# s-esposito/MonoGS

Measured on AMD Instinct MI355X. Metric: rasteriser fwd+bwd Mpix/s @1080p, higher is better.
Workload: dtype f32; 1 GPU; C5: 2000000 Gaussians, 1920x1080, fwd+bwd, seeded synthetic map (SURVEY.md 8d), one keyframe per GPU; gaussians=2000000, width=1920, height=1080, settle_steps=60, instance_count=device-side (capacity mode, overflow checked), parallelism=keyframe-per-gpu x1

## Files before the change

### include/monogs_raster.h

```cpp
#ifndef MONOGS_RASTER_H
#define MONOGS_RASTER_H

#include <stddef.h>
#include <stdint.h>

#ifdef __cplusplus
extern "C" {
#endif

#define MGS_ABI_VERSION 10
#define MGS_TILE 16

typedef struct mgs_camera {
    int32_t image_height;
    int32_t image_width;
    float tanfovx;
    float tanfovy;
    float scale_modifier;
    int32_t sh_degree;
    int32_t sh_coeffs;
    int32_t scale_dim;
    int32_t flags;
    const float* bg;
    const float* viewmatrix;
    const float* projmatrix;
    const float* projmatrix_raw;
    const float* campos;
} mgs_camera;

#define MGS_FLAG_EXCLUSIVE_DEVICE 1

typedef struct mgs_timing {
    float preprocess_ms;
    float depth_sort_ms;
    float scan_ms;
    float duplicate_ms;
    float sort_ms;
    float ranges_ms;
    float blend_fwd_ms;
    float blend_bwd_ms;
    float geom_bwd_ms;
} mgs_timing;

int mgs_abi_version(void);
const char* mgs_last_error(void);

#define MGS_MAX_GAUSSIANS ((1 << 26) - 1)

size_t mgs_geometry_bytes(int32_t P);
size_t mgs_image_bytes(int32_t width, int32_t height);
size_t mgs_binning_bytes(uint64_t num_rendered, int32_t width, int32_t height);
size_t mgs_backward_bytes(int32_t P);
float* mgs_backward_tau(void* backward_scratch, int32_t P);

int mgs_forward_preprocess(const mgs_camera* cam, int32_t P,
                           const float* means3D,
                           const float* shs,
                           const float* colors_precomp,
                           const float* opacities,
                           const float* scales,
                           const float* rotations,
                           const float* cov3D_precomp,
                           void* geometry, int32_t* radii ,
                           void* prepare_backward ,
                           uint64_t* num_rendered ,
                           const uint32_t* prev_status ,
                           uint32_t* prev_status_out ,
                           mgs_timing* timing , void* stream);

int mgs_forward_render(const mgs_camera* cam, int32_t P, uint64_t num_rendered,
                       void* geometry, void* binning, void* image,
                       float* out_color, float* out_depth, float* out_opacity, int32_t* n_touched,
                       uint32_t* status ,
                       mgs_timing* timing, void* stream);

#define MGS_STATUS_CAPACITY_OVERFLOW 1u
#define MGS_STATUS_DEPTH_SORT_TIMEOUT 2u
#define MGS_STATUS_TILE_SORT_TIMEOUT 4u

int mgs_debug_set_radix_spin_limit(uint32_t limit);
int mgs_debug_set_option(const char* name, int64_t value);

int mgs_binning_path(int32_t P, int32_t W, int32_t H);

size_t mgs_debug_sort_temp_bytes(uint64_t n, int32_t bits);
int mgs_debug_sort_pairs(uint32_t* keys, uint32_t* vals, uint32_t* keys_alt, uint32_t* vals_alt, uint64_t n, int32_t bits,
                         void* temp, void* stream);

int mgs_forward_render_capacity(const mgs_camera* cam, int32_t P, uint64_t capacity,
                                void* geometry, void* binning, void* image,
                                float* out_color, float* out_depth, float* out_opacity, int32_t* n_touched,
                                uint32_t* overflow, mgs_timing* timing, void* stream);
int mgs_forward_capacity(const mgs_camera* cam, int32_t P, const float* means3D, const float* shs,
                         const float* colors_precomp, const float* opacities, const float* scales, const float* rotations,
                         const float* cov3D_precomp, void* geometry, int32_t* radii, void* prepare_backward,
                         uint64_t capacity, void* binning, void* image, float* out_color, float* out_depth,
                         float* out_opacity, int32_t* n_touched, uint32_t* overflow, mgs_timing* timing, void* stream);

int mgs_backward(const mgs_camera* cam, int32_t P, uint64_t num_rendered,
                 const float* means3D, const float* shs, const float* colors_precomp,
                 const float* opacities, const float* scales, const float* rotations,
                 const float* cov3D_precomp, const int32_t* radii,
                 const void* geometry, const void* binning, const void* image,
                 const float* dL_dcolor, const float* dL_ddepth,
                 float* dL_dmeans2D,
                 float* dL_dcolors,
                 float* dL_dopacity,
                 float* dL_dmeans3D,
                 float* dL_dcov3D,
                 float* dL_dsh,
                 float* dL_dscales,
                 float* dL_drotations,
                 float* dL_dtau,
                 void* backward_scratch, int32_t scratch_prepared, mgs_timing* timing, void* stream);

#define MGS_VALU_CEILING_BLOCKS 2048
int mgs_debug_valu_ceiling(float* out, int32_t iters, void* stream);

int mgs_debug_set_blend_events(void* fwd_start, void* fwd_end, void* bwd_start, void* bwd_end);

#define MGS_BLEND_STATS_WORDS 24
int mgs_debug_blend_stats(const mgs_camera* cam, int32_t P, uint64_t num_rendered, const void* geometry,
                          const void* binning, const void* image, uint64_t* stats_dev, void* stream);

int mgs_mark_visible(int32_t P, const float* means3D, const float* viewmatrix, const float* projmatrix,
                     uint8_t* visible, void* stream);

size_t mgs_knn_scratch_bytes(int32_t P);
int mgs_dist2_knn(int32_t P, const float* points , float* out ,
                  void* scratch, void* stream);

#define MGS_LOSS_TRACKING 1
#define MGS_LOSS_INVERT_DEPTH 2
#define MGS_LOSS_SCRATCH_DAB 10
#define MGS_LOSS_SCRATCH_LOSS 12
size_t mgs_loss_scratch_bytes(void);
int mgs_loss_forward(int32_t width, int32_t height, int32_t mode, int32_t init, float lambda_rgb,
                     const float* render, const float* depth, const float* opacity, const float* gt_rgb,
                     const float* gt_depth, const uint8_t* mask, const uint8_t* grad_mask,
                     const float* exposure_a, const float* exposure_b, float* scratch, float* loss_out,
                     void* stream);
int mgs_loss_backward(int32_t width, int32_t height, int32_t mode, int32_t init, float lambda_rgb,
                      const float* render, const float* depth, const float* opacity, const float* gt_rgb,
                      const float* gt_depth, const uint8_t* mask, const uint8_t* grad_mask,
                      const float* exposure_a, const float* exposure_b, const float* scratch,
                      const float* grad_out, float* d_render, float* d_depth, float* d_exposure, void* stream);
int mgs_loss_grads(int32_t width, int32_t height, int32_t mode, int32_t init, float lambda_rgb,
                   const float* render, const float* depth, const float* opacity, const float* gt_rgb,
                   const float* gt_depth, const uint8_t* mask, const uint8_t* grad_mask,
                   const float* exposure_a, const float* exposure_b, float* scratch, float* d_render, float* d_depth,
                   void* stream);

#define MGS_POSE_STICKY 1
int mgs_pose_step(float* R, float* T, float* rot_delta, float* trans_delta, float* exposure_a, float* exposure_b,
                  const float* grad_rot, const float* grad_trans, const float* grad_a, const float* grad_b,
                  float* adam_m, float* adam_v, int32_t step, float lr_rot, float lr_trans, float lr_exposure,
                  float beta1, float beta2, float eps, float converged_threshold, int32_t* step_counter, float* out,
                  int32_t flags, float* host_flag ,
                  const float* projmatrix_raw, float* viewmatrix, float* projmatrix, float* campos ,
                  void* stream);
int mgs_pose_step_batch(int32_t n, void* const* ptrs, float lr_rot, float lr_trans, float lr_exposure, float beta1,
                        float beta2, float eps, float converged_threshold, int32_t flags, void* stream);

int mgs_backproject(int32_t N, int32_t W, int32_t H, const int64_t* selected, const float* rgb ,
                    const float* depth , const int32_t* segmentation ,
                    const float* exposure_a, const float* exposure_b, float fx, float fy, float cx, float cy,
                    const float* R, const float* T, float* points , float* features ,
                    int32_t* ids , void* stream);

int mgs_camera_setup(const float* R, const float* T, const float* projmatrix_raw, float* viewmatrix ,
                     float* projmatrix , float* campos , void* stream);

int mgs_adam_step(int32_t n_tensors, float* const* params, const float* const* grads, float* const* exp_avg,
                  float* const* exp_avg_sq, const uint64_t* numel, const float* lr, double beta1, double beta2,
                  double eps, int32_t step, int32_t* step_counter,
                  const float* lr_device ,
                  void* stream);
int mgs_densify_stats(int32_t P, const float* viewspace_grad , const int32_t* radii,
                      float* xyz_gradient_accum , float* denom , float* max_radii_2d ,
                      void* stream);
int mgs_window_stats(int32_t P, int32_t n_keyframes, const float* const* grad_means2D, const int32_t* const* radii,
                     const int32_t* const* n_touched, float* grad_norm , float* visible ,
                     float* max_radii , int32_t accumulate, uint64_t* visibility_bits, void* stream);
int mgs_window_apply(int32_t P, const float* grad_norm, const float* visible, const float* max_radii,
                     float* xyz_gradient_accum, float* denom, float* max_radii_2d, void* stream);
int mgs_lr_schedule_step(int32_t* iteration, float* lr_out, double lr_init, double lr_final, int32_t lr_delay_steps,
                         double lr_delay_mult, int32_t max_steps, void* stream);

int mgs_activate_forward(int32_t P, int32_t scale_dim , const float* rot_raw ,
                         const float* scale_raw , const float* opacity_raw ,
                         float* rotations , float* scales3 , float* opacities ,
                         void* stream);
int mgs_activate_backward(int32_t P, int32_t scale_dim, const float* rot_raw, const float* scales3,
                          const float* opacities, const float* grad_rotations, const float* grad_scales3,
                          const float* grad_opacities, float* d_rot_raw, float* d_scale_raw, float* d_opacity_raw,
                          void* stream);

int mgs_sum_buffers(int32_t n_src, const float* const* src, float* dst, uint64_t count, void* stream);

#ifdef __cplusplus
}
#endif
#endif
```

### monogs_amd/_lib.py

```python
from __future__ import annotations

import ctypes as C
import os

_HERE = os.path.dirname(os.path.abspath(__file__))
LIB_PATH = os.environ.get("MGS_LIB_PATH") or os.path.join(_HERE, "lib", "libmonogs_raster.so")
ABI_VERSION = 10

c_float_p = C.c_void_p


class MgsCamera(C.Structure):
    _fields_ = [
        ("image_height", C.c_int32), ("image_width", C.c_int32),
        ("tanfovx", C.c_float), ("tanfovy", C.c_float), ("scale_modifier", C.c_float),
        ("sh_degree", C.c_int32), ("sh_coeffs", C.c_int32), ("scale_dim", C.c_int32), ("flags", C.c_int32),
        ("bg", C.c_void_p), ("viewmatrix", C.c_void_p), ("projmatrix", C.c_void_p),
        ("projmatrix_raw", C.c_void_p), ("campos", C.c_void_p),
    ]


class MgsTiming(C.Structure):
    _fields_ = [(n, C.c_float) for n in (
        "preprocess_ms", "depth_sort_ms", "scan_ms", "duplicate_ms", "sort_ms", "ranges_ms", "blend_fwd_ms",
        "blend_bwd_ms", "geom_bwd_ms")]

    def as_dict(self):
        return {n: float(getattr(self, n)) for n, _ in self._fields_}


SIGNATURES = {
    "mgs_abi_version": (C.c_int, []),
    "mgs_last_error": (C.c_char_p, []),
    "mgs_geometry_bytes": (C.c_size_t, [C.c_int32]),
    "mgs_image_bytes": (C.c_size_t, [C.c_int32, C.c_int32]),
    "mgs_binning_bytes": (C.c_size_t, [C.c_uint64, C.c_int32, C.c_int32]),
    "mgs_backward_bytes": (C.c_size_t, [C.c_int32]),
    "mgs_forward_preprocess": (C.c_int, [C.POINTER(MgsCamera), C.c_int32] + [C.c_void_p] * 7
                               + [C.c_void_p, C.c_void_p, C.c_void_p, C.POINTER(C.c_uint64), C.c_void_p, C.POINTER(C.c_uint32),
                                  C.POINTER(MgsTiming), C.c_void_p]),
    "mgs_forward_capacity": (C.c_int, [C.POINTER(MgsCamera), C.c_int32] + [C.c_void_p] * 7 + [C.c_void_p] * 3 + [C.c_uint64]
                             + [C.c_void_p] * 7 + [C.POINTER(MgsTiming), C.c_void_p]),
    "mgs_forward_render": (C.c_int, [C.POINTER(MgsCamera), C.c_int32, C.c_uint64] + [C.c_void_p] * 8
                           + [C.POINTER(MgsTiming), C.c_void_p]),
    "mgs_debug_set_radix_spin_limit": (C.c_int, [C.c_uint32]),
    "mgs_debug_set_option": (C.c_int, [C.c_char_p, C.c_int64]),
    "mgs_binning_path": (C.c_int, [C.c_int32, C.c_int32, C.c_int32]),
    "mgs_debug_sort_temp_bytes": (C.c_size_t, [C.c_uint64, C.c_int32]),
    "mgs_debug_sort_pairs": (C.c_int, [C.c_void_p] * 4 + [C.c_uint64, C.c_int32, C.c_void_p, C.c_void_p]),
    "mgs_forward_render_capacity": (C.c_int, [C.POINTER(MgsCamera), C.c_int32, C.c_uint64] + [C.c_void_p] * 8
                                    + [C.POINTER(MgsTiming), C.c_void_p]),
    "mgs_backward": (C.c_int, [C.POINTER(MgsCamera), C.c_int32, C.c_uint64] + [C.c_void_p] * 7
                     + [C.c_void_p] * 4 + [C.c_void_p] * 2 + [C.c_void_p] * 9
                     + [C.c_void_p, C.c_int32, C.POINTER(MgsTiming), C.c_void_p]),
    "mgs_backward_tau": (C.c_void_p, [C.c_void_p, C.c_int32]),
    "mgs_debug_blend_stats": (C.c_int, [C.POINTER(MgsCamera), C.c_int32, C.c_uint64] + [C.c_void_p] * 5),
    "mgs_debug_valu_ceiling": (C.c_int, [C.c_void_p, C.c_int32, C.c_void_p]),
    "mgs_debug_set_blend_events": (C.c_int, [C.c_void_p] * 4),
    "mgs_mark_visible": (C.c_int, [C.c_int32, C.c_void_p, C.c_void_p, C.c_void_p, C.c_void_p, C.c_void_p]),
    "mgs_loss_scratch_bytes": (C.c_size_t, []),
    "mgs_loss_forward": (C.c_int, [C.c_int32] * 4 + [C.c_float] + [C.c_void_p] * 9 + [C.c_void_p, C.c_void_p, C.c_void_p]),
    "mgs_loss_backward": (C.c_int, [C.c_int32] * 4 + [C.c_float] + [C.c_void_p] * 9
                          + [C.c_void_p, C.c_void_p, C.c_void_p, C.c_void_p, C.c_void_p, C.c_void_p]),
    "mgs_loss_grads": (C.c_int, [C.c_int32] * 4 + [C.c_float] + [C.c_void_p] * 9 + [C.c_void_p] * 4),
    "mgs_backproject": (C.c_int, [C.c_int32] * 3 + [C.c_void_p] * 6 + [C.c_float] * 4 + [C.c_void_p] * 6),
    "mgs_camera_setup": (C.c_int, [C.c_void_p] * 7),
    "mgs_pose_step": (C.c_int, [C.c_void_p] * 12 + [C.c_int32] + [C.c_float] * 7
                      + [C.c_void_p, C.c_void_p, C.c_int32, C.c_void_p] + [C.c_void_p] * 4 + [C.c_void_p]),
    "mgs_pose_step_batch": (C.c_int, [C.c_int32, C.POINTER(C.c_void_p)] + [C.c_float] * 7 + [C.c_int32, C.c_void_p]),
    "mgs_adam_step": (C.c_int, [C.c_int32] + [C.c_void_p] * 6 + [C.c_double] * 3 + [C.c_int32, C.c_void_p, C.c_void_p, C.c_void_p]),
    "mgs_window_stats": (C.c_int, [C.c_int32, C.c_int32] + [C.c_void_p] * 6 + [C.c_int32, C.c_void_p, C.c_void_p]),
    "mgs_window_apply": (C.c_int, [C.c_int32] + [C.c_void_p] * 7),
    "mgs_lr_schedule_step": (C.c_int, [C.c_void_p, C.c_void_p, C.c_double, C.c_double, C.c_int32, C.c_double, C.c_int32, C.c_void_p]),
    "mgs_densify_stats": (C.c_int, [C.c_int32] + [C.c_void_p] * 6),
    "mgs_sum_buffers": (C.c_int, [C.c_int32, C.POINTER(C.c_void_p), C.c_void_p, C.c_uint64, C.c_void_p]),
    "mgs_activate_forward": (C.c_int, [C.c_int32, C.c_int32] + [C.c_void_p] * 7),
    "mgs_activate_backward": (C.c_int, [C.c_int32, C.c_int32] + [C.c_void_p] * 10),
    "mgs_knn_scratch_bytes": (C.c_size_t, [C.c_int32]),
    "mgs_dist2_knn": (C.c_int, [C.c_int32, C.c_void_p, C.c_void_p, C.c_void_p, C.c_void_p]),
}

_lib = None


class MonoGSNativeError(RuntimeError):
    pass


def load():
    global _lib
    if _lib is not None:
        return _lib
    if not os.path.exists(LIB_PATH):
        raise MonoGSNativeError(
            f"{LIB_PATH} not found: build it with `python -c 'import __graft_entry__ as g; g.build()'` "
            "or `make -C monogs_amd/csrc`.  There is no CPU fallback.")
    lib = C.CDLL(LIB_PATH)
    for name, (res, args) in SIGNATURES.items():
        fn = getattr(lib, name)
        fn.restype = res
        fn.argtypes = args
    if lib.mgs_abi_version() != ABI_VERSION:
        raise MonoGSNativeError(f"ABI mismatch: library {lib.mgs_abi_version()} vs binding {ABI_VERSION}; rebuild")
    for kv in filter(None, os.environ.get("MGS_DEBUG_OPTIONS", "").split(",")):
        k, _, v = kv.partition("=")
        if lib.mgs_debug_set_option(k.strip().encode(), int(v)) != 0:
            raise MonoGSNativeError(f"MGS_DEBUG_OPTIONS: {lib.mgs_last_error().decode()}")
    _lib = lib
    return lib


def check(rc: int, what: str):
    if rc != 0:
        msg = load().mgs_last_error().decode("utf-8", "replace")
        raise Exception(msg) if rc == 1 else MonoGSNativeError(f"{what}: {msg}")
```

### monogs_amd/csrc/api.hip

```cpp
#include "common.h"

#include <stdarg.h>
#include <stdio.h>
#include <string.h>

namespace mgs {

static thread_local char g_err[512] = "";

void set_error(const char* fmt, ...) {
    va_list ap;
    va_start(ap, fmt);
    vsnprintf(g_err, sizeof(g_err), fmt, ap);
    va_end(ap);
}

static inline char* take(char*& p, size_t bytes) {
    char* r = p;
    p += align_up(bytes, 256);
    return r;
}

GeometryState GeometryState::carve(void* base, int P) {
    char* p = (char*)align_up((size_t)base, 256);
    GeometryState g;
    g.rec = (float*)take(p, (size_t)P * REC_FLOATS * sizeof(float));
    g.depth_key = (uint32_t*)take(p, (size_t)P * sizeof(uint32_t));
    g.depth_alt = (uint32_t*)take(p, (size_t)P * sizeof(uint32_t));
    g.iota = (uint32_t*)take(p, (size_t)P * sizeof(uint32_t));
    g.iota_alt = (uint32_t*)take(p, (size_t)P * sizeof(uint32_t));
    g.perm = (uint32_t*)take(p, (size_t)P * sizeof(uint32_t));
    g.point_offsets = (uint32_t*)take(p, (size_t)P * sizeof(uint32_t));
    g.scan_blocks = (uint32_t*)take(p, ((size_t)scan_nblocks(P) + 64) * sizeof(uint32_t));
    g.clamped = (uint8_t*)take(p, (size_t)P * 4);
    g.rect = (uint2*)take(p, (size_t)P * sizeof(uint2));
    g.rect_sorted = (uint2*)take(p, (size_t)P * sizeof(uint2));
    g.scan_status = (uint64_t*)take(p, (SCAN_SMALL_MAX_BLOCKS + 1) * sizeof(uint64_t));
    g.tile_hist = (uint32_t*)take(p, 4 * 256 * sizeof(uint32_t));
    g.sort_temp_bytes = radix_depth_temp_bytes((uint64_t)P);
    g.sort_temp = take(p, g.sort_temp_bytes);
    g.end = p;
    return g;
}
size_t GeometryState::bytes(int P) {
    const GeometryState g = carve(nullptr, P);
    return (size_t)g.end + 256;
}

size_t ImageState::bytes(int W, int H) {
    const size_t HW = (size_t)W * H, nt = (size_t)tiles_x(W) * tiles_y(H);
    return align_up(HW * 4, 256) * 2 + align_up(nt * sizeof(uint2), 256) + 256;
}
ImageState ImageState::carve(void* base, int W, int H) {
    const size_t HW = (size_t)W * H, nt = (size_t)tiles_x(W) * tiles_y(H);
    char* p = (char*)align_up((size_t)base, 256);
    ImageState s;
    s.final_T = (float*)take(p, HW * 4);
    s.n_contrib = (uint32_t*)take(p, HW * 4);
    s.ranges = (uint2*)take(p, nt * sizeof(uint2));
    return s;
}

size_t BinningState::bytes(uint64_t R, int W, int H) {
    const size_t r = (size_t)(R ? R : 1);
    return align_up(r * 4, 256) * 4 + align_up(mgs::sort_temp_bytes(R, tile_bits(W, H)), 256) + 256 + 256;
}
BinningState BinningState::carve(void* base, uint64_t R, int W, int H) {
    const size_t r = (size_t)(R ? R : 1);
    char* p = (char*)align_up((size_t)base, 256);
    BinningState b;
    b.keys_a = (uint32_t*)take(p, r * 4);
    b.keys_b = (uint32_t*)take(p, r * 4);
    b.vals_a = (uint32_t*)take(p, r * 4);
    b.vals_b = (uint32_t*)take(p, r * 4);
    const bool in_b = radix_result_in_b(tile_bits(W, H));
    b.keys_sorted = in_b ? b.keys_b : b.keys_a;
    b.vals_sorted = in_b ? b.vals_b : b.vals_a;
    b.sort_temp_bytes = mgs::sort_temp_bytes(R, tile_bits(W, H));
    b.sort_temp = take(p, b.sort_temp_bytes);
    b.count = (uint32_t*)take(p, 2 * sizeof(uint32_t));
    return b;
}

struct StageTimer {
    hipStream_t s;
    bool on;
    hipEvent_t ev[10];
    int n = 0;
    StageTimer(hipStream_t s_, bool on_) : s(s_), on(on_) {
        if (on) for (auto& e : ev) (void)hipEventCreate(&e);
    }
    ~StageTimer() {
        if (on) for (auto& e : ev) (void)hipEventDestroy(e);
    }
    void mark() {
        if (on && n < 10) (void)hipEventRecord(ev[n++], s);
    }
    float ms(int i) {
        float t = 0.f;
        if (on && i + 1 < n) (void)hipEventElapsedTime(&t, ev[i], ev[i + 1]);
        return t;
    }
    void sync() {
        if (on && n) (void)hipEventSynchronize(ev[n - 1]);
    }
};

static int check_cam(const mgs_camera* cam) {
    if (!cam) { set_error("camera is NULL"); return 1; }
    if (cam->image_width <= 0 || cam->image_height <= 0) { set_error("image size must be positive"); return 1; }
    if (!cam->bg || !cam->viewmatrix || !cam->projmatrix || !cam->projmatrix_raw || !cam->campos) {
        set_error("camera tensors (bg, viewmatrix, projmatrix, projmatrix_raw, campos) must be non-NULL");
        return 1;
    }
    return 0;
}

static hipEvent_t g_dbg_fwd_events[2] = {nullptr, nullptr}, g_dbg_bwd_events[2] = {nullptr, nullptr};

static int check_map_size(int32_t P) {
    if (P > MGS_MAX_GAUSSIANS) {
        set_error("P exceeds MGS_MAX_GAUSSIANS (2^26 - 1): the gradient-line offset of the blend backward is 32-bit");
        return 1;
    }
    return 0;
}

}

using namespace mgs;

extern "C" {

int mgs_abi_version(void) { return MGS_ABI_VERSION; }
int mgs_binning_path(int32_t P, int32_t W, int32_t H) { return binning_path(P, W, H); }
const char* mgs_last_error(void) { return g_err; }

size_t mgs_geometry_bytes(int32_t P) { return GeometryState::bytes(P < 0 ? 0 : P); }
size_t mgs_image_bytes(int32_t W, int32_t H) { return ImageState::bytes(W, H); }
size_t mgs_binning_bytes(uint64_t R, int32_t W, int32_t H) { return BinningState::bytes(R, W, H); }
size_t mgs_backward_bytes(int32_t P) {
    return (size_t)(P < 0 ? 0 : P) * GRAD_FLOATS * sizeof(float) + (size_t)(TAU_SLOTS + 1) * 16 * sizeof(float) + 256;
}
float* mgs_backward_tau(void* backward_scratch, int32_t P) { return backward_tau_out(backward_scratch, P < 0 ? 0 : P); }

int mgs_forward_preprocess(const mgs_camera* cam, int32_t P, const float* means3D, const float* shs,
                           const float* colors_precomp, const float* opacities, const float* scales,
                           const float* rotations, const float* cov3D_precomp, void* geometry, int32_t* radii,
                           void* prepare_backward, uint64_t* num_rendered, const uint32_t* prev_status,
                           uint32_t* prev_status_out, mgs_timing* timing, void* stream) {
    if (check_cam(cam)) return 1;
    if (P < 0) { set_error("P must be >= 0"); return 1; }
    if (check_map_size(P)) return 1;
    if (num_rendered) *num_rendered = 0;
    if (prev_status_out) *prev_status_out = 0;
    if (P == 0) {
        if (prev_status && prev_status_out) {
            MGS_HIP(hipMemcpyAsync(prev_status_out, prev_status, sizeof(uint32_t), hipMemcpyDeviceToHost, (hipStream_t)stream));
            MGS_HIP(hipStreamSynchronize((hipStream_t)stream));
        }
        return 0;
    }
    if (!means3D || !opacities || !geometry || !radii) { set_error("means3D, opacities, geometry, radii must be non-NULL"); return 1; }
    if ((shs == nullptr) == (colors_precomp == nullptr)) {
        set_error("Please provide excatly one of either SHs or precomputed colors!");
        return 1;
    }
    const bool have_sr = scales != nullptr || rotations != nullptr;
    if ((have_sr && (!scales || !rotations || cov3D_precomp)) || (!have_sr && !cov3D_precomp)) {
        set_error("Please provide exactly one of either scale/rotation pair or precomputed 3D covariance!");
        return 1;
    }
    if (shs && (cam->sh_degree < 0 || cam->sh_degree > 3 || cam->sh_coeffs < (cam->sh_degree + 1) * (cam->sh_degree + 1))) {
        set_error("sh_degree must be 0..3 and shs must hold at least (degree+1)^2 coefficients");
        return 1;
    }
    hipStream_t s = (hipStream_t)stream;
    GeometryState g = GeometryState::carve(geometry, P);
    StageTimer tm(s, timing != nullptr);
    tm.mark();
    if (int rc = launch_preprocess_forward(*cam, P, means3D, shs, colors_precomp, opacities, scales, rotations,
                                           cov3D_precomp, g, radii,
                                           prepare_backward ? backward_grad_acc(prepare_backward) : nullptr, s)) return rc;
    tm.mark();
    const bool exclusive = (cam->flags & MGS_FLAG_EXCLUSIVE_DEVICE) != 0;
    const bool per_tile = binning_path(P, cam->image_width, cam->image_height) != 0;
    if (per_tile) {
        tm.mark();
        if (int rc = launch_scan(g, P, s, exclusive, g.rect)) return rc;
    } else if (depth_chain_is_small(P)) {
        if (int rc = launch_depth_chain_small(g, P, s)) return rc;
        tm.mark();
    } else {
        if (int rc = launch_depth_sort(g, P, depth_sort_payload(P, cam->image_width, cam->image_height), s, exclusive)) return rc;
        tm.mark();
        if (int rc = launch_scan(g, P, s, exclusive, g.rect_sorted)) return rc;
    }
    tm.mark();
    if (num_rendered) {
        uint32_t total = 0, sort_errors[RADIX_ERROR_WORDS] = {0, 0, 0, 0};
        MGS_HIP(hipMemcpyAsync(&total, g.scan_blocks + scan_nblocks(P), sizeof(uint32_t), hipMemcpyDeviceToHost, s));
        MGS_HIP(hipMemcpyAsync(sort_errors, radix_depth_error_flag(g.sort_temp, (uint64_t)P), sizeof(sort_errors),
                               hipMemcpyDeviceToHost, s));
        if (prev_status && prev_status_out)
            MGS_HIP(hipMemcpyAsync(prev_status_out, prev_status, sizeof(uint32_t), hipMemcpyDeviceToHost, s));
        MGS_HIP(hipStreamSynchronize(s));
        if (sort_errors[0] | sort_errors[1] | sort_errors[2] | sort_errors[3]) { set_error("depth sort: a look-back spin timed out (results invalid)"); return 3; }
        *num_rendered = total;
    }
    if (timing) {
        if (!num_rendered) MGS_HIP(hipStreamSynchronize(s));
        timing->preprocess_ms = tm.ms(0);
        timing->depth_sort_ms = per_tile ? 0.f : tm.ms(1);
        timing->scan_ms = tm.ms(2);
    }
    return 0;
}

static int g_opt_tile_sort_fused = 1;

static int forward_render_impl(const mgs_camera* cam, int32_t P, uint64_t R, bool capacity, void* geometry,
                               void* binning, void* image, float* out_color, float* out_depth, float* out_opacity,
                               int32_t* n_touched, uint32_t* overflow, mgs_timing* timing, void* stream) {
    if (check_cam(cam)) return 1;
    if (P < 0) { set_error("P must be >= 0"); return 1; }
    if (check_map_size(P)) return 1;
    if (!image || !out_color || !out_depth || !out_opacity) { set_error("image scratch and outputs must be non-NULL"); return 1; }
    if (P > 0 && (!geometry || !n_touched)) { set_error("geometry and n_touched must be non-NULL"); return 1; }
    if (R > 0 && !binning) { set_error("binning scratch is NULL"); return 1; }
    if (R >= (1ull << 32)) { set_error("num_rendered exceeds 2^32-1"); return 1; }
    if (P == 0) R = 0;
    hipStream_t s = (hipStream_t)stream;
    const int W = cam->image_width, H = cam->image_height;
    GeometryState g = GeometryState::carve(geometry, P);
    ImageState img = ImageState::carve(image, W, H);
    BinningState b = BinningState::carve(binning, R, W, H);
    const uint32_t* n_dev = nullptr;
    StageTimer tm(s, timing != nullptr);
    const bool cap = capacity && binning;
    if (cap) n_dev = b.count;
    const bool per_tile = binning_path(P, W, H) != 0;
    tm.mark();
    if (int rc = launch_duplicate(*cam, P, g, b, capacity ? R : (R > 0 ? 0xFFFFFFFFull : 0ull), n_touched, img, R,
                                  tile_bits(W, H), cap ? b.count : nullptr, overflow, s, per_tile)) return rc;
    tm.mark();
    if (int rc = launch_sort(g, b, R, tile_bits(W, H), s, n_dev, (cam->flags & MGS_FLAG_EXCLUSIVE_DEVICE) != 0, img.ranges,
                             per_tile)) return rc;
    const uint32_t* sort_err = R > 0 ? radix_error_flag(b.sort_temp, R, tile_bits(W, H)) : nullptr;
    const bool sort_tiles = per_tile && R > 0;
    const TileSortArgs ts = sort_tiles ? tile_sort_args(*cam, g, b, R, n_dev) : TileSortArgs{};
    const bool fused = sort_tiles && g_opt_tile_sort_fused != 0;
    if (sort_tiles && !fused)
        if (int rc = launch_tile_depth_sort(*cam, ts, img, sort_err, s)) return rc;
    tm.mark();
    if (g_dbg_fwd_events[0]) MGS_HIP(hipEventRecord(g_dbg_fwd_events[0], s));
    if (int rc = launch_blend_forward(*cam, g, b, img, out_color, out_depth, out_opacity, n_touched, sort_err, overflow,
                                      fused ? &ts : nullptr, s)) return rc;
    if (g_dbg_fwd_events[1]) MGS_HIP(hipEventRecord(g_dbg_fwd_events[1], s));
    tm.mark();
    if (timing) {
        tm.sync();
        timing->duplicate_ms = tm.ms(0);
        timing->sort_ms = tm.ms(1);
        timing->ranges_ms = 0.f;
        timing->blend_fwd_ms = tm.ms(2);
    }
    return 0;
}

int mgs_forward_render(const mgs_camera* cam, int32_t P, uint64_t R, void* geometry, void* binning, void* image,
                       float* out_color, float* out_depth, float* out_opacity, int32_t* n_touched,
                       uint32_t* status, mgs_timing* timing, void* stream) {
    return forward_render_impl(cam, P, R, false, geometry, binning, image, out_color, out_depth, out_opacity, n_touched,
                               status, timing, stream);
}

int mgs_forward_render_capacity(const mgs_camera* cam, int32_t P, uint64_t capacity, void* geometry, void* binning,
                                void* image, float* out_color, float* out_depth, float* out_opacity,
                                int32_t* n_touched, uint32_t* overflow, mgs_timing* timing, void* stream) {
    if (capacity == 0) { set_error("capacity must be > 0"); return 1; }
    return forward_render_impl(cam, P, capacity, true, geometry, binning, image, out_color, out_depth, out_opacity,
                               n_touched, overflow, timing, stream);
}

int mgs_forward_capacity(const mgs_camera* cam, int32_t P, const float* means3D, const float* shs,
                         const float* colors_precomp, const float* opacities, const float* scales, const float* rotations,
                         const float* cov3D_precomp, void* geometry, int32_t* radii, void* prepare_backward,
                         uint64_t capacity, void* binning, void* image, float* out_color, float* out_depth,
                         float* out_opacity, int32_t* n_touched, uint32_t* overflow, mgs_timing* timing, void* stream) {
    if (int rc = mgs_forward_preprocess(cam, P, means3D, shs, colors_precomp, opacities, scales, rotations, cov3D_precomp,
                                        geometry, radii, prepare_backward, nullptr, nullptr, nullptr, timing, stream)) return rc;
    return mgs_forward_render_capacity(cam, P, capacity, geometry, binning, image, out_color, out_depth, out_opacity,
                                       n_touched, overflow, timing, stream);
}

int mgs_backward(const mgs_camera* cam, int32_t P, uint64_t R, const float* means3D, const float* shs,
                 const float* colors_precomp, const float* opacities, const float* scales, const float* rotations,
                 const float* cov3D_precomp, const int32_t* radii, const void* geometry, const void* binning,
                 const void* image, const float* dL_dcolor, const float* dL_ddepth, float* dL_dmeans2D,
                 float* dL_dcolors, float* dL_dopacity, float* dL_dmeans3D, float* dL_dcov3D, float* dL_dsh,
                 float* dL_dscales, float* dL_drotations, float* dL_dtau, void* backward_scratch,
                 int32_t scratch_prepared, mgs_timing* timing, void* stream) {
    if (check_cam(cam)) return 1;
    if (P < 0) { set_error("P must be >= 0"); return 1; }
    if (check_map_size(P)) return 1;
    hipStream_t s = (hipStream_t)stream;
    if (P == 0) {
        if (dL_dtau) MGS_HIP(zero_fill(dL_dtau, 6 * sizeof(float), s));
        return 0;
    }
    if (!means3D || !opacities || !radii || !geometry || !image || !dL_dcolor || !dL_ddepth || !backward_scratch) {
        set_error("means3D, opacities, radii, geometry, image, dL_dcolor, dL_ddepth, backward_scratch must be non-NULL");
        return 1;
    }
    if (R > 0 && !binning) { set_error("binning scratch is NULL"); return 1; }
    const int W = cam->image_width, H = cam->image_height;
    GeometryState g = GeometryState::carve(const_cast<void*>(geometry), P);
    ImageState img = ImageState::carve(const_cast<void*>(image), W, H);
    BinningState b = BinningState::carve(const_cast<void*>(binning), R, W, H);
    float* grad_acc = backward_grad_acc(backward_scratch);
    StageTimer tm(s, timing != nullptr);
    float* tau_part = (dL_dtau && (P + 255) / 256 > TAU_DIRECT_MAX_BLOCKS) ? backward_tau_part(backward_scratch, P) : nullptr;
    if (scratch_prepared) {
        if (dL_dtau && dL_dtau != backward_tau_out(backward_scratch, P)) {
            set_error("scratch_prepared: dL_dtau must be mgs_backward_tau(backward_scratch, P)");
            return 1;
        }
    } else {
        MGS_HIP(zero_fill2(grad_acc, (size_t)P * GRAD_FLOATS * sizeof(float) + (tau_part ? (size_t)TAU_SLOTS * 16 * sizeof(float) : 0),
                           dL_dtau, 6 * sizeof(float), s));
    }
    tm.mark();
    if (R > 0) {
        const bool pose_only = !dL_dcolors && !dL_dopacity && !dL_dsh && !shs;
        if (g_dbg_bwd_events[0]) MGS_HIP(hipEventRecord(g_dbg_bwd_events[0], s));
        if (int rc = launch_blend_backward(*cam, g, b, img, dL_dcolor, dL_ddepth, grad_acc, pose_only, s)) return rc;
        if (g_dbg_bwd_events[1]) MGS_HIP(hipEventRecord(g_dbg_bwd_events[1], s));
    }
    tm.mark();
    GeomBackwardArgs a;
    a.means3D = means3D; a.shs = shs; a.colors_precomp = colors_precomp; a.opacities = opacities;
    a.scales = scales; a.rotations = rotations; a.cov3D_precomp = cov3D_precomp; a.radii = radii;
    a.grad_acc = grad_acc;
    a.dL_dmeans2D = dL_dmeans2D; a.dL_dcolors = dL_dcolors; a.dL_dopacity = dL_dopacity;
    a.dL_dmeans3D = dL_dmeans3D; a.dL_dcov3D = dL_dcov3D; a.dL_dsh = dL_dsh; a.dL_dscales = dL_dscales;
    a.dL_drotations = dL_drotations; a.dL_dtau = dL_dtau; a.tau_part = tau_part;
    if (int rc = launch_geom_backward(*cam, P, g, a, s)) return rc;
    tm.mark();
    if (timing) {
        tm.sync();
        timing->blend_bwd_ms = tm.ms(0);
        timing->geom_bwd_ms = tm.ms(1);
    }
    return 0;
}

int mgs_debug_blend_stats(const mgs_camera* cam, int32_t P, uint64_t R, const void* geometry, const void* binning,
                           const void* image, uint64_t* stats_dev, void* stream) {
    if (check_cam(cam)) return 1;
    if (!geometry || !image || !stats_dev || (R > 0 && !binning)) { set_error("bad arguments"); return 1; }
    hipStream_t s = (hipStream_t)stream;
    MGS_HIP(zero_fill(stats_dev, MGS_BLEND_STATS_WORDS * sizeof(uint64_t), s));
    if (P == 0 || R == 0) return 0;
    const int W = cam->image_width, H = cam->image_height;
    GeometryState g = GeometryState::carve(const_cast<void*>(geometry), P);
    ImageState img = ImageState::carve(const_cast<void*>(image), W, H);
    BinningState b = BinningState::carve(const_cast<void*>(binning), R, W, H);
    return launch_blend_backward_stats(*cam, g, b, img, (unsigned long long*)stats_dev, s);
}

int mgs_debug_valu_ceiling(float* out, int32_t iters, void* stream) {
    if (!out || iters < 1) { set_error("mgs_debug_valu_ceiling: bad arguments"); return 1; }
    return launch_valu_ceiling(out, iters, (hipStream_t)stream);
}

int mgs_debug_set_radix_spin_limit(uint32_t limit) { return set_radix_spin_limit(limit); }

int mgs_debug_set_blend_events(void* fwd_start, void* fwd_end, void* bwd_start, void* bwd_end) {
    if ((fwd_start == nullptr) != (fwd_end == nullptr) || (bwd_start == nullptr) != (bwd_end == nullptr)) {
        set_error("mgs_debug_set_blend_events: a pair is both events or neither");
        return 1;
    }
    g_dbg_fwd_events[0] = (hipEvent_t)fwd_start; g_dbg_fwd_events[1] = (hipEvent_t)fwd_end;
    g_dbg_bwd_events[0] = (hipEvent_t)bwd_start; g_dbg_bwd_events[1] = (hipEvent_t)bwd_end;
    return 0;
}

static int g_opt_debug_sort_exclusive = 0;
size_t mgs_debug_sort_temp_bytes(uint64_t n, int32_t bits) { return radix_temp_bytes(n, bits); }
int mgs_debug_sort_pairs(uint32_t* keys, uint32_t* vals, uint32_t* keys_alt, uint32_t* vals_alt, uint64_t n, int32_t bits,
                         void* temp, void* stream) {
    if (bits < 1 || bits > 32 || (n && (!keys || !vals || !keys_alt || !vals_alt || !temp))) {
        set_error("mgs_debug_sort_pairs: bad arguments");
        return 1;
    }
    if (n == 0) return 0;
    hipStream_t s = (hipStream_t)stream;
    if (int rc = radix_sort_pairs(keys, vals, keys_alt, vals_alt, n, bits, temp, s, nullptr, false, nullptr, nullptr, nullptr, false,
                                  g_opt_debug_sort_exclusive != 0))
        return rc;
    if (radix_result_in_b(bits)) {
        MGS_HIP(hipMemcpyAsync(keys, keys_alt, n * 4, hipMemcpyDeviceToDevice, s));
        MGS_HIP(hipMemcpyAsync(vals, vals_alt, n * 4, hipMemcpyDeviceToDevice, s));
    }
    uint32_t err[RADIX_ERROR_WORDS];
    MGS_HIP(hipMemcpyAsync(err, radix_error_flag(temp, n, bits), sizeof(err), hipMemcpyDeviceToHost, s));
    MGS_HIP(hipStreamSynchronize(s));
    if (err[0] | err[1] | err[2] | err[3]) { set_error("mgs_debug_sort_pairs: a look-back spin timed out"); return 2; }
    return 0;
}

int mgs_debug_set_option(const char* name, int64_t value) {
    if (name && !strcmp(name, "radix_scanned")) { g_opt_radix_scanned = (int)value; return 0; }
    if (name && !strcmp(name, "radix_ballot_rank")) { g_opt_radix_ballot_rank = (int)value; return 0; }
    if (name && !strcmp(name, "radix_tile_items")) { g_opt_radix_tile_items = (int)value; return 0; }
    if (name && !strcmp(name, "radix_xcd_band")) { g_opt_radix_xcd_band = (int)value; return 0; }
    if (name && !strcmp(name, "debug_sort_exclusive")) { g_opt_debug_sort_exclusive = (int)value; return 0; }
    if (name && !strcmp(name, "dup_slot_major")) { g_opt_dup_slot_major = (int)value; return 0; }
    if (name && !strcmp(name, "blend_bwd_transposed")) { g_opt_blend_bwd_transposed = (int)value; return 0; }
    if (name && !strcmp(name, "scan_small")) { g_opt_scan_small = (int)value; return 0; }
    if (name && !strcmp(name, "depth_small")) { g_opt_depth_small = (int)value; return 0; }
    if (name && !strcmp(name, "tile_sort_fused")) { g_opt_tile_sort_fused = value < 0 ? 1 : (int)value; return 0; }
    if (name && !strcmp(name, "blend_lds_pad_fwd")) { g_opt_blend_lds_pad_fwd = (int)value; return 0; }
    if (name && !strcmp(name, "blend_lds_pad_bwd")) { g_opt_blend_lds_pad_bwd = (int)value; return 0; }
    if (name && !strcmp(name, "knn_grid_min")) { g_opt_knn_grid_min = value > 0x7FFFFFFF ? 0x7FFFFFFF : (int)value; return 0; }
    set_error("mgs_debug_set_option: unknown option");
    return 1;
}

int mgs_mark_visible(int32_t P, const float* means3D, const float* viewmatrix, const float* projmatrix,
                     uint8_t* visible, void* stream) {
    (void)projmatrix;
    if (P < 0 || (P > 0 && (!means3D || !viewmatrix || !visible))) { set_error("bad arguments"); return 1; }
    return launch_mark_visible(P, means3D, viewmatrix, visible, (hipStream_t)stream);
}

size_t mgs_knn_scratch_bytes(int32_t P) { return knn_scratch_bytes(P); }

int mgs_dist2_knn(int32_t P, const float* points, float* out, void* scratch, void* stream) {
    if (P < 0 || (P > 0 && (!points || !out))) { set_error("bad arguments"); return 1; }
    return launch_knn(P, points, out, scratch, (hipStream_t)stream);
}

}
```

### monogs_amd/csrc/blend.hip

```cpp
#include "common.h"
#include "tile_sort.h"

#include <type_traits>


namespace mgs {

extern int g_opt_blend_lds_pad_fwd, g_opt_blend_lds_pad_bwd;
#ifdef BS_TRACE
static unsigned long long* g_trace_fwd = nullptr;
static unsigned long long* g_trace_bwd = nullptr;
#define BS_STAMP(v) asm volatile("s_memrealtime %0\n\ts_waitcnt lgkmcnt(0)" : "=s"(v) :: "memory")
#endif

__device__ __forceinline__ uint32_t bcast(uint32_t v, int lane) {
    return (uint32_t)__builtin_amdgcn_readlane((int)v, lane);
}

constexpr int MGS_WG_WAVES = 4;
#define MGS_TILE_WAVE(ntiles_, tile_, wave_, ws_)                                                   \
    const int tile_ = (int)blockIdx.x, wave_ = __builtin_amdgcn_readfirstlane((int)(threadIdx.x >> 6)), ws_ = wave_; \
    if (tile_ >= (ntiles_)) return;
struct BlendArgs {
#ifdef BS_TRACE
    unsigned long long* trace;
#endif
    const float4* __restrict__ rec;
    const uint32_t* __restrict__ point_list;
    const uint2* __restrict__ ranges;
    const float* __restrict__ bg;
    int W, H, gx;
};

__device__ __forceinline__ bool quadrant_hit(const float4 c , const float4 n ,
                                             float qx0, float qy0, unsigned long long alive) {
    const float x0 = qx0 - 0.05f - c.x, x1 = qx0 + (float)(SUB - 1) + 0.05f - c.x;
    const float y0 = qy0 - 0.05f - c.y, y1 = qy0 + (float)(SUB - 1) + 0.05f - c.y;
    if (c.z < 0.f) return false;
    if (!((c.z >= x0) && (-c.z <= x1) && (c.w >= y0) && (-c.w <= y1))) return false;
    {
        const int ix0 = (int)fminf(8.f, fmaxf(0.f, ceilf(-x0 - c.z - 0.06f))), ix1 = (int)fminf(7.f, fmaxf(-1.f, floorf(-x0 + c.z + 0.06f)));
        const int iy0 = (int)fminf(8.f, fmaxf(0.f, ceilf(-y0 - c.w - 0.06f))), iy1 = (int)fminf(7.f, fmaxf(-1.f, floorf(-y0 + c.w + 0.06f)));
        if (ix0 > ix1 || iy0 > iy1) return false;
        const unsigned long long cols = (unsigned long long)((0xFFu >> (7 - ix1)) & (0xFFu << ix0) & 0xFFu) * 0x0101010101010101ull;
        const unsigned long long rows = (~0ull >> (8 * (7 - iy1))) & (~0ull << (8 * iy0));
        if ((cols & rows & alive) == 0ull) return false;
    }
    if (x0 <= 0.f && x1 >= 0.f && y0 <= 0.f && y1 >= 0.f) return true;
    if (!(n.x > 0.f) || !(n.z > 0.f)) return true;
    const float rby = -n.y * __builtin_amdgcn_rcpf(n.z), rbx = -n.y * __builtin_amdgcn_rcpf(n.x);
    auto edge_x = [&](float xe) {
        const float t = fminf(y1, fmaxf(y0, rby * xe));
        return n.x * xe * xe + 2.f * n.y * xe * t + n.z * t * t;
    };
    auto edge_y = [&](float ye) {
        const float t = fminf(x1, fmaxf(x0, rbx * ye));
        return n.x * t * t + 2.f * n.y * t * ye + n.z * ye * ye;
    };
    const float qmin = fminf(fminf(edge_x(x0), edge_x(x1)), fminf(edge_y(y0), edge_y(y1)));
    return qmin <= 1.02f;
}

struct Rec {
    float px, py, ca, cb, cc, op, r, g, b, z;
};
__device__ __forceinline__ Rec fetch(const BlendArgs& a, uint32_t gid_uniform) {
    const const_float_p p = MGS_CONST(reinterpret_cast<const float*>(a.rec)) + (size_t)gid_uniform * REC_FLOATS;
    return Rec{p[R_X], p[R_Y], p[R_CA], p[R_CB], p[R_CC], p[R_OPAC], p[R_R], p[R_G], p[R_B], p[R_DEPTH]};
}

#ifdef MGS_FWD_SCALAR
#define MGS_RECOP "s"
#else
#define MGS_RECOP "v"
#endif
template <bool TOUCH>
__device__ __forceinline__ void blend_one(unsigned long long& live, unsigned long long& mask, float& T, uint32_t& last, float& C0, float& C1, float& C2,
                                      float& D, const Rec& g, float power, float alpha, uint32_t pos, int j,
                                      int& touched_cnt) {
    const float test_T = T * (1.f - alpha);
    float w;
    int cnt;
    if (TOUCH) {
        asm volatile(
            "s_mov_b64 exec, %[live]\n\t"
            "v_cmpx_nlt_f32_e32 vcc, 0, %[power]\n\t"
            "v_cmpx_ngt_f32_e32 vcc, %[amin], %[alpha]\n\t"
            "v_cmp_gt_f32_e32 vcc, %[tmin], %[tt]\n\t"
            "s_andn2_b64 exec, exec, vcc\n\t"
            "s_andn2_b64 %[live], %[live], vcc\n\t"
            "s_cselect_b64 %[mask], %[mask], 0\n\t"
            "v_mul_f32_e32 %[w], %[alpha], %[T]\n\t"
            "v_mov_b32_e32 %[T], %[tt]\n\t"
            "v_mov_b32_e32 %[last], %[pos]\n\t"
            "v_cmp_lt_f32_e32 vcc, 0.5, %[tt]\n\t"
            "v_fmac_f32_e32 %[C0], %[cr], %[w]\n\t"
            "v_fmac_f32_e32 %[C1], %[cg], %[w]\n\t"
            "s_bcnt1_i32_b64 %[cnt], vcc\n\t"
            "s_mov_b32 m0, %[j]\n\t"
            "v_fmac_f32_e32 %[C2], %[cb], %[w]\n\t"
            "v_fmac_f32_e32 %[D], %[cz], %[w]\n\t"
            "s_mov_b64 exec, -1\n\t"
            "v_writelane_b32 %[tc], %[cnt], m0\n\t"
            : [live] "+s"(live), [mask] "+s"(mask), [T] "+v"(T), [last] "+v"(last), [C0] "+v"(C0), [C1] "+v"(C1), [C2] "+v"(C2), [D] "+v"(D),
              [w] "=&v"(w), [cnt] "=&s"(cnt), [tc] "+v"(touched_cnt)
            : [power] "v"(power), [alpha] "v"(alpha), [tt] "v"(test_T), [amin] "s"(1.0f / 255.0f), [tmin] "s"(0.0001f),
              [pos] "s"(pos), [cr] MGS_RECOP(g.r), [cg] MGS_RECOP(g.g), [cb] MGS_RECOP(g.b), [cz] MGS_RECOP(g.z), [j] "s"(j)
            : "vcc", "scc", "m0");
    } else {
        asm volatile(
            "s_mov_b64 exec, %[live]\n\t"
            "v_cmpx_nlt_f32_e32 vcc, 0, %[power]\n\t"
            "v_cmpx_ngt_f32_e32 vcc, %[amin], %[alpha]\n\t"
            "v_cmp_gt_f32_e32 vcc, %[tmin], %[tt]\n\t"
            "s_andn2_b64 exec, exec, vcc\n\t"
            "s_andn2_b64 %[live], %[live], vcc\n\t"
            "s_cselect_b64 %[mask], %[mask], 0\n\t"
            "v_mul_f32_e32 %[w], %[alpha], %[T]\n\t"
            "v_mov_b32_e32 %[T], %[tt]\n\t"
            "v_mov_b32_e32 %[last], %[pos]\n\t"
            "v_fmac_f32_e32 %[C0], %[cr], %[w]\n\t"
            "v_fmac_f32_e32 %[C1], %[cg], %[w]\n\t"
            "v_fmac_f32_e32 %[C2], %[cb], %[w]\n\t"
            "v_fmac_f32_e32 %[D], %[cz], %[w]\n\t"
            "s_mov_b64 exec, -1\n\t"
            : [live] "+s"(live), [mask] "+s"(mask), [T] "+v"(T), [last] "+v"(last), [C0] "+v"(C0), [C1] "+v"(C1), [C2] "+v"(C2), [D] "+v"(D),
              [w] "=&v"(w)
            : [power] "v"(power), [alpha] "v"(alpha), [tt] "v"(test_T), [amin] "s"(1.0f / 255.0f), [tmin] "s"(0.0001f),
              [pos] "s"(pos), [cr] MGS_RECOP(g.r), [cg] MGS_RECOP(g.g), [cb] MGS_RECOP(g.b), [cz] MGS_RECOP(g.z)
            : "vcc", "scc");
    }
}

template <bool SORT>
__global__ void __launch_bounds__(256) blend_forward_kernel(BlendArgs a, float* __restrict__ out_color,
                                                            float* __restrict__ out_depth,
                                                            float* __restrict__ out_opacity,
                                                            float* __restrict__ final_T,
                                                            uint32_t* __restrict__ n_contrib,
                                                            int32_t* __restrict__ n_touched,
                                                            uint2* ranges_rw ,
                                                            const uint32_t* __restrict__ sort_err,
                                                            uint32_t* __restrict__ status, TileSortArgs ts) {
    MGS_TILE_WAVE(a.gx * ((a.H + TILE - 1) / TILE), tile, wave, ws)
    const int tx = tile % a.gx, ty = tile / a.gx;
    const int lane = threadIdx.x & 63;
    const bool first_of_tile = wave == 0 && lane == 0;
    const int qx0i = tx * TILE + (wave & 1) * SUB, qy0i = ty * TILE + (wave >> 1) * SUB;
    const int pxi = qx0i + (lane & 7), pyi = qy0i + (lane >> 3);
    const bool inside = pxi < a.W && pyi < a.H;
    const float pxf = (float)pxi, pyf = (float)pyi;
    const float qx0 = (float)qx0i, qy0 = (float)qy0i;
    uint2 range = ranges_rw[tile];
    const uint2 range_raw = range;
    const bool sort_bad = sort_err != nullptr && radix_failed(sort_err) != 0u;
    {
        if (sort_bad && tile == 0 && first_of_tile && status) atomicOr(status, (uint32_t)MGS_STATUS_TILE_SORT_TIMEOUT);
        if (sort_bad || range.x >= range.y) {
            range = make_uint2(0u, 0u);
            if (first_of_tile) ranges_rw[tile] = range;
        }
    }

    float T = 1.f, C0 = 0.f, C1 = 0.f, C2 = 0.f, D = 0.f;
    uint32_t last = 0;
    unsigned long long live = __builtin_amdgcn_ballot_w64(inside);
#ifdef BS_TRACE
    unsigned long long tr0;
    BS_STAMP(tr0);
#endif

    uint32_t gid_n = 0;
    float4 box_n = make_float4(0.f, 0.f, -1.f, -1.f), ell_n = make_float4(0.f, 0.f, 0.f, 0.f);
#ifdef MGS_FWD_SCALAR
    typedef float fv2 __attribute__((ext_vector_type(2)));
    typedef float fv8 __attribute__((ext_vector_type(8)));
    const const_float_p recs = MGS_CONST(reinterpret_cast<const float*>(a.rec));
    auto prefetch = [&](uint32_t i) {
        gid_n = 0;
        box_n = make_float4(0.f, 0.f, -1.f, -1.f);
        if (i < range.y) {
            gid_n = a.point_list[i];
            box_n = a.rec[(size_t)gid_n * 4];
            ell_n = a.rec[(size_t)gid_n * 4 + 3];
        }
    };
    auto walk_step = [&](auto touch_tag, uint32_t base, uint32_t gid_l, unsigned long long mask) {
        int touched_cnt = 0;
        const uint32_t goff_l = gid_l << 6;
        while (mask) {
            int j;
            asm volatile("s_ff1_i32_b64 %0, %1\n\ts_bitset0_b64 %1, %0" : "=&s"(j), "+s"(mask));
            const uint32_t goff = (uint32_t)__builtin_amdgcn_readlane((int)goff_l, j);
            fv2 r0;
            fv8 r1;
            asm volatile("s_load_dwordx2 %0, %2, %3\n\ts_load_dwordx8 %1, %2, %3 offset:0x10\n\ts_waitcnt lgkmcnt(0)"
                         : "=&s"(r0), "=&s"(r1) : "s"(recs), "s"(goff) : "memory");
            const Rec g{r0[0], r0[1], r1[0], r1[1], r1[2], r1[3], r1[4], r1[5], r1[6], r1[7]};
            const float dx = g.px - pxf, dy = g.py - pyf;
            const float power = dx * (g.ca * dx + g.cb * dy) + (g.cc * dy) * dy;
            const float alpha = fminf(0.99f, g.op * __builtin_amdgcn_exp2f(power));
            blend_one<decltype(touch_tag)::value>(live, mask, T, last, C0, C1, C2, D, g, power, alpha,
                                                  (base - range.x) + (uint32_t)j + 1u, j, touched_cnt);
        }
        if (decltype(touch_tag)::value && touched_cnt != 0) atomicAdd(n_touched + gid_l, touched_cnt);
    };
    if (range.x < range.y) prefetch(range.x + lane);
    for (uint32_t base = range.x; base < range.y && live != 0ull; base += WAVE) {
        const uint32_t gid_l = gid_n;
        const float4 c = box_n, el = ell_n;
        prefetch(base + WAVE + lane);
        const unsigned long long mask = __builtin_amdgcn_ballot_w64(quadrant_hit(c, el, qx0, qy0, live));
        if ((live & __builtin_amdgcn_ballot_w64(T > 0.5f)) != 0ull) walk_step(std::true_type{}, base, gid_l, mask);
        else walk_step(std::false_type{}, base, gid_l, mask);
    }
#else
    __shared__ __attribute__((aligned(16))) float4 s_queue[MGS_WG_WAVES][WAVE][3];
    __shared__ uint32_t s_list[TDS_CAP], s_wsum[TDS_WAVES], s_red[2 * TDS_WAVES];
    static_assert(sizeof(s_queue) == sizeof(uint32_t) * (TDS_CAP + TDS_WAVES * TDS_RADIX), "sort scratch = record queue");
    bool list_in_lds = false;
    if constexpr (SORT) {
        uint32_t* const s_k = reinterpret_cast<uint32_t*>(&s_queue[0][0][0]);
        const uint32_t n_lds = tile_depth_sort(ts, range_raw, sort_bad,
                                               TdsLds{s_k, s_list, reinterpret_cast<uint32_t (*)[TDS_RADIX]>(s_k + TDS_CAP),
                                                      s_wsum, s_red});
        list_in_lds = n_lds != 0u && n_lds == range.y - range.x;
        if (!list_in_lds) __syncthreads();
    }
    float4 c1_n = make_float4(0.f, 0.f, 0.f, 0.f), c2_n = c1_n;
    float4* const my_entry = &s_queue[ws][lane][0];
    const uint32_t q_base = (uint32_t)__builtin_amdgcn_readfirstlane((int)(uint32_t)(uintptr_t)&s_queue[ws][0][0]);
    auto prefetch = [&](uint32_t i) {
        gid_n = 0;
        box_n = make_float4(0.f, 0.f, -1.f, -1.f);
        if (i < range.y) {
            if constexpr (SORT) gid_n = list_in_lds ? s_list[i - range.x] : ts.vals[i];
            else gid_n = a.point_list[i];
            box_n = a.rec[(size_t)gid_n * 4];
            ell_n = a.rec[(size_t)gid_n * 4 + 3];
            c1_n = a.rec[(size_t)gid_n * 4 + 1];
            c2_n = a.rec[(size_t)gid_n * 4 + 2];
        }
    };
    auto walk_step = [&](auto touch_tag, uint32_t base, uint32_t gid_l, unsigned long long mask) {
        int touched_cnt = 0;
        while (mask) {
            const int j = __builtin_ctzll(mask);
            mask &= ~(1ull << j);
            typedef float qv2 __attribute__((ext_vector_type(2)));
            typedef float qv4 __attribute__((ext_vector_type(4)));
            qv2 e0;
            qv4 e1, e2;
            {
                const uint32_t ad = q_base + (uint32_t)j * 48u;
                asm volatile("ds_read_b64 %0, %3\n\tds_read_b128 %1, %3 offset:16\n\tds_read_b128 %2, %3 offset:32"
                             : "=&v"(e0), "=&v"(e1), "=&v"(e2) : "v"(ad) : "memory");
            }
            asm volatile("s_waitcnt lgkmcnt(2)" : "+v"(e0));
            float dx = e0[0] - pxf, dy = e0[1] - pyf;
            asm volatile("s_waitcnt lgkmcnt(1)" : "+v"(e1), "+v"(dx), "+v"(dy));
            const float power = dx * (e1[0] * dx + e1[1] * dy) + (e1[2] * dy) * dy;
            float alpha = fminf(0.99f, e1[3] * __builtin_amdgcn_exp2f(power));
            asm volatile("s_waitcnt lgkmcnt(0)" : "+v"(e2), "+v"(alpha));
            const Rec g{e0[0], e0[1], e1[0], e1[1], e1[2], e1[3], e2[0], e2[1], e2[2], e2[3]};
            blend_one<decltype(touch_tag)::value>(live, mask, T, last, C0, C1, C2, D, g, power, alpha,
                                                  (base - range.x) + (uint32_t)j + 1u, j, touched_cnt);
        }
        if (decltype(touch_tag)::value && touched_cnt != 0) atomicAdd(n_touched + gid_l, touched_cnt);
    };
    if (range.x < range.y) prefetch(range.x + lane);
    for (uint32_t base = range.x; base < range.y && live != 0ull; base += WAVE) {
        const uint32_t gid_l = gid_n;
        const float4 c = box_n, el = ell_n;
        my_entry[0] = c; my_entry[1] = c1_n; my_entry[2] = c2_n;
        prefetch(base + WAVE + lane);
        const unsigned long long mask = __builtin_amdgcn_ballot_w64(quadrant_hit(c, el, qx0, qy0, live));
        if ((live & __builtin_amdgcn_ballot_w64(T > 0.5f)) != 0ull) walk_step(std::true_type{}, base, gid_l, mask);
        else walk_step(std::false_type{}, base, gid_l, mask);
    }
#endif
#ifdef BS_TRACE
    if (a.trace) {
        unsigned long long tr1;
        BS_STAMP(tr1);
        const unsigned hw = __builtin_amdgcn_s_getreg((31 << 11) | 4), xcc = __builtin_amdgcn_s_getreg((31 << 11) | 20);
        if (lane == 0) {
            unsigned long long* o = a.trace + ((size_t)tile * 4 + wave) * 4;
            o[0] = tr0; o[1] = tr1; o[2] = (unsigned long long)hw | ((unsigned long long)xcc << 32); o[3] = range.y - range.x;
        }
    }
#endif
    if (inside) {
        const size_t pix = (size_t)pyi * a.W + pxi, HW = (size_t)a.H * a.W;
        final_T[pix] = T;
        n_contrib[pix] = last;
        out_color[pix] = C0 + T * a.bg[0];
        out_color[HW + pix] = C1 + T * a.bg[1];
        out_color[2 * HW + pix] = C2 + T * a.bg[2];
        out_depth[pix] = D;
        out_opacity[pix] = 1.f - T;
    }
}

static BlendArgs make_args(const mgs_camera& cam, const GeometryState& g, const BinningState& b,
                           const ImageState& img) {
    BlendArgs a;
#ifdef BS_TRACE
    a.trace = nullptr;
#endif
    a.rec = reinterpret_cast<const float4*>(g.rec);
    a.point_list = b.vals_sorted;
    a.ranges = img.ranges;
    a.bg = cam.bg;
    a.W = cam.image_width;
    a.H = cam.image_height;
    a.gx = tiles_x(a.W);
    return a;
}

int launch_blend_forward(const mgs_camera& cam, const GeometryState& g, const BinningState& b,
                         const ImageState& img, float* out_color, float* out_depth, float* out_opacity,
                         int32_t* n_touched, const uint32_t* sort_err, uint32_t* status, const TileSortArgs* tile_sort,
                         hipStream_t s) {
    BlendArgs a = make_args(cam, g, b, img);
#ifdef BS_TRACE
    a.trace = g_trace_fwd;
#endif
    const int ntiles = a.gx * tiles_y(a.H);
    if (ntiles == 0) return 0;
    const dim3 grid(ntiles), block(256);
    const TileSortArgs ts = tile_sort ? *tile_sort : TileSortArgs{};
#ifdef MGS_FWD_SCALAR
    if (tile_sort)
        if (int rc = launch_tile_depth_sort(cam, ts, img, sort_err, s)) return rc;
    hipLaunchKernelGGL(blend_forward_kernel<false>, grid, block, (size_t)g_opt_blend_lds_pad_fwd, s, a, out_color, out_depth,
                       out_opacity, img.final_T, img.n_contrib, n_touched, img.ranges, sort_err, status, ts);
#else
    if (tile_sort)
        hipLaunchKernelGGL(blend_forward_kernel<true>, grid, block, (size_t)g_opt_blend_lds_pad_fwd, s, a, out_color, out_depth,
                           out_opacity, img.final_T, img.n_contrib, n_touched, img.ranges, sort_err, status, ts);
    else
        hipLaunchKernelGGL(blend_forward_kernel<false>, grid, block, (size_t)g_opt_blend_lds_pad_fwd, s, a, out_color, out_depth,
                           out_opacity, img.final_T, img.n_contrib, n_touched, img.ranges, sort_err, status, ts);
#endif
    MGS_HIP(hipGetLastError());
    return 0;
}


__device__ __forceinline__ float swap32_add(float x, float y) {
    auto r = __builtin_amdgcn_permlane32_swap(__float_as_uint(x), __float_as_uint(y), false, false);
    return __uint_as_float(r[0]) + __uint_as_float(r[1]);
}
__device__ __forceinline__ float swap16_add(float x, float y) {
    auto r = __builtin_amdgcn_permlane16_swap(__float_as_uint(x), __float_as_uint(y), false, false);
    return __uint_as_float(r[0]) + __uint_as_float(r[1]);
}
template <int XOR>
__device__ __forceinline__ float swz_add(float v) {
    return v + __int_as_float(__builtin_amdgcn_ds_swizzle(__float_as_int(v), 0x001F | (XOR << 10)));
}
__device__ __forceinline__ float row_sum_all(float v) {
    v = swz_add<1>(v);
    v = swz_add<2>(v);
    v = swz_add<4>(v);
    v = swz_add<8>(v);
    return v;
}
__device__ __forceinline__ int reduce10_slot(int lane) {
    const int row = lane >> 4, pos = lane & 15;
    if (pos == 15) return row == 0 ? 0 : row == 1 ? 2 : row == 2 ? 1 : 3;
    if (pos == 0) return row == 0 ? 4 : row == 1 ? 6 : row == 2 ? 5 : 7;
    if (pos == 1) return row == 0 ? 8 : row == 2 ? 9 : -1;
    return -1;
}
__device__ __forceinline__ float reduce10(float a0, float a1, float a2, float a3, float a4, float a5, float a6,
                                          float a7, float a8, float a9, int lane) {
    const float b0 = swap32_add(a0, a1), b1 = swap32_add(a2, a3), b2 = swap32_add(a4, a5);
    const float b3 = swap32_add(a6, a7), b4 = swap32_add(a8, a9);
    float c0 = swap16_add(b0, b1);
    float c1 = swap16_add(b2, b3);
    float c2 = swz_add<16>(b4);
    c0 = row_sum_all(c0);
    c1 = row_sum_all(c1);
    c2 = row_sum_all(c2);
    const int pos = lane & 15;
    return pos == 15 ? c0 : (pos == 0 ? c1 : c2);
}

__device__ __forceinline__ int reduce6_slot(int lane) {
    const int row = lane >> 4, pos = lane & 15;
    if (pos == 15) return row == 0 ? G_SX : row == 1 ? G_SXX : row == 2 ? G_SY : G_SXY;
    if (pos == 0) return row == 0 ? G_SYY : row == 2 ? G_DDEPTH : -1;
    return -1;
}
__device__ __forceinline__ float reduce6(float a0, float a1, float a2, float a3, float a4, float a5, int lane) {
    const float b0 = swap32_add(a0, a1), b1 = swap32_add(a2, a3), b2 = swap32_add(a4, a5);
    float c0 = swap16_add(b0, b1);
    float c1 = swz_add<16>(b2);
    c0 = row_sum_all(c0);
    c1 = row_sum_all(c1);
    return (lane & 15) == 15 ? c0 : c1;
}

__device__ __forceinline__ uint32_t wave_max_u32(uint32_t v) {
#pragma unroll
    for (int o = 32; o > 0; o >>= 1) v = max(v, (uint32_t)__shfl_xor((int)v, o, 64));
    return v;
}

template <bool POSE_ONLY>
__global__ void __launch_bounds__(256) blend_backward_kernel(BlendArgs a, int ntiles,
                                                             const float* __restrict__ final_T,
                                                             const uint32_t* __restrict__ n_contrib,
                                                             const float* __restrict__ dL_dcolor,
                                                             const float* __restrict__ dL_ddepth,
                                                             float* __restrict__ grad_acc) {
    const int wave = threadIdx.x >> 6, lane = threadIdx.x & 63;
    const int tile = (int)blockIdx.x;
    if (tile >= ntiles) return;
    const int tx = tile % a.gx, ty = tile / a.gx;
    const uint2 range = a.ranges[tile];
    if (range.y <= range.x) return;
    const size_t HW = (size_t)a.H * a.W;
    const float bg0 = a.bg[0], bg1 = a.bg[1], bg2 = a.bg[2];

    const int qx0i = tx * TILE + (wave & 1) * SUB, qy0i = ty * TILE + (wave >> 1) * SUB;
    const int pxi = qx0i + (lane & 7), pyi = qy0i + (lane >> 3);
    const bool inside = pxi < a.W && pyi < a.H;
    const size_t pix = (size_t)pyi * a.W + pxi;
    const float pxf = (float)pxi, pyf = (float)pyi, qx0 = (float)qx0i, qy0 = (float)qy0i;
    const float T_final = inside ? final_T[pix] : 0.f;
    const uint32_t last = inside ? n_contrib[pix] : 0u;
    const float g0 = inside ? dL_dcolor[pix] : 0.f;
    const float g1 = inside ? dL_dcolor[HW + pix] : 0.f;
    const float g2 = inside ? dL_dcolor[2 * HW + pix] : 0.f;
    const float gd = inside ? dL_ddepth[pix] : 0.f;
    const float bgT = -T_final * (bg0 * g0 + bg1 * g1 + bg2 * g2);
    float T = T_final, Bk = 0.f;
    const uint32_t maxc = wave_max_u32(last);
    if (maxc == 0) return;
    const uint32_t end = range.x + maxc;

    const int slot = POSE_ONLY ? reduce6_slot(lane) : reduce10_slot(lane);
    const uint32_t slot_bytes = slot < 0 ? 0u : (uint32_t)slot * 4u;

    uint32_t gid_n = 0;
    float4 box_n = make_float4(0.f, 0.f, -1.f, -1.f), ell_n = make_float4(0.f, 0.f, 0.f, 0.f);
    auto prefetch = [&](int b) {
        gid_n = 0;
        box_n = make_float4(0.f, 0.f, -1.f, -1.f);
        const uint32_t i = range.x + (uint32_t)b * WAVE + lane;
        if (b >= 0 && i < end) {
            gid_n = a.point_list[i];
            box_n = a.rec[(size_t)gid_n * 4];
            ell_n = a.rec[(size_t)gid_n * 4 + 3];
        }
    };
    prefetch((int)((maxc - 1) / WAVE));
    for (int b = (int)((maxc - 1) / WAVE); b >= 0; --b) {
        const uint32_t gid_l = gid_n;
        const float4 c = box_n, el = ell_n;
        prefetch(b - 1);
        const unsigned long long alive = __builtin_amdgcn_ballot_w64(last >= (uint32_t)b * WAVE + 1u);
        unsigned long long mask = __builtin_amdgcn_ballot_w64(quadrant_hit(c, el, qx0, qy0, alive));
        const int rel_last = (int)last - (int)((uint32_t)b * WAVE + 1u);
        while (mask) {
            const int j = 63 - __builtin_clzll(mask);
            mask &= ~(1ull << j);
            const uint32_t gid = bcast(gid_l, j);
            const Rec g = fetch(a, gid);
            const float dx = g.px - pxf, dy = g.py - pyf;
            const float power = dx * (g.ca * dx + g.cb * dy) + (g.cc * dy) * dy;
            const float G = __builtin_amdgcn_exp2f(power);
            const float alpha = fminf(0.99f, g.op * G);
            const bool act = (j <= rel_last) && !(power > 0.f) && !(alpha < 1.0f / 255.0f);
            if (__builtin_amdgcn_ballot_w64(act) == 0ull) continue;
            const float a_eff = act ? alpha : 0.f;
            const float inv = __builtin_amdgcn_rcpf(1.f - a_eff);
            const float Tn = T * inv;
            const float qq = __builtin_fmaf(g.z, gd, __builtin_fmaf(g.b, g2, __builtin_fmaf(g.g, g1, g.r * g0)));
            const float diff = qq - Bk;
            const float dL_dalpha = diff * Tn + bgT * inv;
            Bk = Bk + a_eff * diff;
            T = Tn;
            const float w = a_eff * Tn;
            const float h = act ? G * dL_dalpha : 0.f;
            const float hx = h * dx, hy = h * dy;
            const float s_x = hx, s_y = hy, s_xx = hx * dx, s_xy = hx * dy, s_yy = hy * dy, s_h = h;
            const float s_r = w * g0, s_g = w * g1, s_b = w * g2, s_z = w * gd;
            const float m = POSE_ONLY ? reduce6(s_x, s_y, s_xx, s_xy, s_yy, s_z, lane)
                                      : reduce10(s_x, s_y, s_xx, s_xy, s_yy, s_h, s_r, s_g, s_b, s_z, lane);
            float* const line = grad_acc + (size_t)gid * GRAD_FLOATS;
            if (slot >= 0) asm volatile("global_atomic_add_f32 %0, %1, %2" ::"v"(slot_bytes), "v"(m), "s"(line) : "memory");
        }
    }
}

constexpr int BT_SLOTS = 4;
constexpr int BS_STRIDE = 272;
constexpr int BS_W_OFF = 1280;
constexpr int BS_META_OFF = BS_W_OFF + BT_SLOTS * BS_STRIDE;
__device__ __forceinline__ int bt_slot10(int t) {
    const int bank = t >> 2, m = t & 3;
    if (m == 0) return bank == 3 ? 0 : bank == 1 ? 1 : bank == 2 ? 2 : 3;
    if (m == 1) return bank == 3 ? 4 : bank == 1 ? 5 : bank == 2 ? 6 : 7;
    if (m == 2) return bank == 3 ? 8 : bank == 1 ? 9 : -1;
    return -1;
}
__device__ __forceinline__ int bt_slot6(int t) {
    const int bank = t >> 2, m = t & 3;
    if (m == 0) return bank == 3 ? G_SX : bank == 1 ? G_SY : bank == 2 ? G_SXX : G_SXY;
    if (m == 1) return bank == 3 ? G_SYY : bank == 1 ? G_DDEPTH : -1;
    return -1;
}
__device__ __forceinline__ float reduce_rows10(float v0, float v1, float v2, float v3, float v4, float v5, float v6,
                                               float v7, float v8, float v9, unsigned long long m1, unsigned long long m2) {
    float a0, a1, a2, a3, a4;
    asm volatile(
        "s_nop 1\n\t"
        "v_add_f32_dpp %0, %5, %5 row_ror:8 row_mask:0xf bank_mask:0xc\n\t"
        "v_add_f32_dpp %1, %7, %7 row_ror:8 row_mask:0xf bank_mask:0xc\n\t"
        "v_add_f32_dpp %2, %9, %9 row_ror:8 row_mask:0xf bank_mask:0xc\n\t"
        "v_add_f32_dpp %3, %11, %11 row_ror:8 row_mask:0xf bank_mask:0xc\n\t"
        "v_add_f32_dpp %4, %13, %13 row_ror:8 row_mask:0xf bank_mask:0xc\n\t"
        "v_add_f32_dpp %0, %6, %6 row_ror:8 row_mask:0xf bank_mask:0x3\n\t"
        "v_add_f32_dpp %1, %8, %8 row_ror:8 row_mask:0xf bank_mask:0x3\n\t"
        "v_add_f32_dpp %2, %10, %10 row_ror:8 row_mask:0xf bank_mask:0x3\n\t"
        "v_add_f32_dpp %3, %12, %12 row_ror:8 row_mask:0xf bank_mask:0x3\n\t"
        "v_add_f32_dpp %4, %14, %14 row_ror:8 row_mask:0xf bank_mask:0x3\n\t"
        "v_add_f32_dpp %5, %0, %0 row_half_mirror row_mask:0xf bank_mask:0xa\n\t"
        "v_add_f32_dpp %6, %2, %2 row_half_mirror row_mask:0xf bank_mask:0xa\n\t"
        "v_add_f32_dpp %5, %1, %1 row_half_mirror row_mask:0xf bank_mask:0x5\n\t"
        "v_add_f32_dpp %6, %3, %3 row_half_mirror row_mask:0xf bank_mask:0x5\n\t"
        "v_add_f32_dpp %7, %4, %4 row_half_mirror row_mask:0xf bank_mask:0xf\n\t"
        "v_add_f32_dpp %0, %5, %5 quad_perm:[2,3,0,1] row_mask:0xf bank_mask:0xf\n\t"
        "v_add_f32_dpp %1, %6, %6 quad_perm:[2,3,0,1] row_mask:0xf bank_mask:0xf\n\t"
        "v_add_f32_dpp %2, %7, %7 quad_perm:[2,3,0,1] row_mask:0xf bank_mask:0xf\n\t"
        "v_add_f32_dpp %5, %0, %0 quad_perm:[1,0,3,2] row_mask:0xf bank_mask:0xf\n\t"
        "v_add_f32_dpp %6, %1, %1 quad_perm:[1,0,3,2] row_mask:0xf bank_mask:0xf\n\t"
        "v_add_f32_dpp %7, %2, %2 quad_perm:[1,0,3,2] row_mask:0xf bank_mask:0xf\n\t"
        : "=&v"(a0), "=&v"(a1), "=&v"(a2), "=&v"(a3), "=&v"(a4), "+v"(v0), "+v"(v1), "+v"(v2), "+v"(v3), "+v"(v4), "+v"(v5),
          "+v"(v6), "+v"(v7), "+v"(v8), "+v"(v9));
    const float r12 = __builtin_amdgcn_inverse_ballot_w64(m1) ? v1 : v2;
    return __builtin_amdgcn_inverse_ballot_w64(m2) ? v0 : r12;
}
__device__ __forceinline__ float reduce_rows6(float v0, float v1, float v2, float v3, float v4, float v5,
                                              unsigned long long m2) {
    float a0, a1, a2;
    asm volatile(
        "s_nop 1\n\t"
        "v_add_f32_dpp %0, %3, %3 row_ror:8 row_mask:0xf bank_mask:0xc\n\t"
        "v_add_f32_dpp %1, %5, %5 row_ror:8 row_mask:0xf bank_mask:0xc\n\t"
        "v_add_f32_dpp %2, %7, %7 row_ror:8 row_mask:0xf bank_mask:0xc\n\t"
        "v_add_f32_dpp %0, %4, %4 row_ror:8 row_mask:0xf bank_mask:0x3\n\t"
        "v_add_f32_dpp %1, %6, %6 row_ror:8 row_mask:0xf bank_mask:0x3\n\t"
        "v_add_f32_dpp %2, %8, %8 row_ror:8 row_mask:0xf bank_mask:0x3\n\t"
        "v_add_f32_dpp %3, %0, %0 row_half_mirror row_mask:0xf bank_mask:0xa\n\t"
        "v_add_f32_dpp %3, %1, %1 row_half_mirror row_mask:0xf bank_mask:0x5\n\t"
        "v_add_f32_dpp %4, %2, %2 row_half_mirror row_mask:0xf bank_mask:0xf\n\t"
        "s_nop 1\n\t"
        "v_add_f32_dpp %0, %3, %3 quad_perm:[2,3,0,1] row_mask:0xf bank_mask:0xf\n\t"
        "v_add_f32_dpp %1, %4, %4 quad_perm:[2,3,0,1] row_mask:0xf bank_mask:0xf\n\t"
        "s_nop 0\n\t"
        "v_add_f32_dpp %3, %0, %0 quad_perm:[1,0,3,2] row_mask:0xf bank_mask:0xf\n\t"
        "v_add_f32_dpp %4, %1, %1 quad_perm:[1,0,3,2] row_mask:0xf bank_mask:0xf\n\t"
        : "=&v"(a0), "=&v"(a1), "=&v"(a2), "+v"(v0), "+v"(v1), "+v"(v2), "+v"(v3), "+v"(v4), "+v"(v5));
    return __builtin_amdgcn_inverse_ballot_w64(m2) ? v0 : v1;
}

struct __attribute__((aligned(16))) BtMetaRec { float x, y; uint32_t g; };
struct BtLane {
    const float* fac;
    const float* pix;
    const BtMetaRec* meta;
    int lane;
    float qx0, qy0;
    uint32_t slot_bytes;
    unsigned long long m_out, m_q0, m_q1;
    float* grad_acc;
    int qxi = 0, qyi = 0;
};
template <bool POSE_ONLY, bool WIDE_META = false>
__device__ __forceinline__ void bt_flush(const BtLane L, int n) {
    int lane = L.lane;
    asm volatile("" : "+v"(lane));
    const int q = lane & 15, row = lane >> 4;
    const float* const hp = WIDE_META ? L.fac + row * (BS_STRIDE / 4) + 4 * q : L.fac + 4 * lane;
    const float4 h4 = *reinterpret_cast<const float4*>(hp);
    const float4 w4 = *reinterpret_cast<const float4*>(hp + (WIDE_META ? BS_W_OFF / 4 : BT_SLOTS * WAVE));
    const BtMetaRec me = L.meta[WIDE_META ? row * (BS_STRIDE / 16) : row];
    const float* const fp = L.pix + q * 4;
    float u0, v0;
    if (WIDE_META) {
        int oqx = L.qxi, oqy = L.qyi;
        asm volatile("" : "+s"(oqx), "+s"(oqy));
        u0 = (float)(oqx + 4 * (q & 1)), v0 = (float)(oqy + (q >> 1));
    } else {
        u0 = L.qx0 + (float)(4 * (q & 1)), v0 = L.qy0 + (float)(q >> 1);
    }
    const float dy = me.y - v0;
    const float dx0 = me.x - u0, dx1 = dx0 - 1.f, dx2 = dx0 - 2.f, dx3 = dx0 - 3.f;
    const float hx0 = h4.x * dx0, hx1 = h4.y * dx1, hx2 = h4.z * dx2, hx3 = h4.w * dx3;
    const float H0 = (h4.x + h4.y) + (h4.z + h4.w);
    const float H1 = (hx0 + hx1) + (hx2 + hx3);
    const float H2 = __builtin_fmaf(hx3, dx3, __builtin_fmaf(hx2, dx2, __builtin_fmaf(hx1, dx1, hx0 * dx0)));
    const float s_y = dy * H0, s_xy = dy * H1, s_yy = dy * s_y;
    float m;
    if (POSE_ONLY) {
        const float4 c3 = *reinterpret_cast<const float4*>(fp);
        const float s_z = __builtin_fmaf(w4.w, c3.w, __builtin_fmaf(w4.z, c3.z, __builtin_fmaf(w4.y, c3.y, w4.x * c3.x)));
        m = reduce_rows6(H1, s_y, H2, s_xy, s_yy, s_z, L.m_q0);
    } else {
        const float4 c0 = *reinterpret_cast<const float4*>(fp), c1 = *reinterpret_cast<const float4*>(fp + 64),
                     c2 = *reinterpret_cast<const float4*>(fp + 128), c3 = *reinterpret_cast<const float4*>(fp + 192);
        const float s_r = __builtin_fmaf(w4.w, c0.w, __builtin_fmaf(w4.z, c0.z, __builtin_fmaf(w4.y, c0.y, w4.x * c0.x)));
        const float s_g = __builtin_fmaf(w4.w, c1.w, __builtin_fmaf(w4.z, c1.z, __builtin_fmaf(w4.y, c1.y, w4.x * c1.x)));
        const float s_b = __builtin_fmaf(w4.w, c2.w, __builtin_fmaf(w4.z, c2.z, __builtin_fmaf(w4.y, c2.y, w4.x * c2.x)));
        const float s_z = __builtin_fmaf(w4.w, c3.w, __builtin_fmaf(w4.z, c3.z, __builtin_fmaf(w4.y, c3.y, w4.x * c3.x)));
        m = reduce_rows10(H1, s_y, H2, s_xy, s_yy, H0, s_r, s_g, s_b, s_z, L.m_q1, L.m_q0);
    }
    const unsigned long long rows = n >= BT_SLOTS ? ~0ull : ((1ull << (16 * n)) - 1ull);
    const uint32_t off = (WIDE_META ? me.g : me.g * (uint32_t)(GRAD_FLOATS * sizeof(float))) + L.slot_bytes;
    if (__builtin_amdgcn_inverse_ballot_w64(L.m_out & rows))
        asm volatile("global_atomic_add_f32 %0, %1, %2" ::"v"(off), "v"(m), "s"(L.grad_acc) : "memory");
}

template <bool POSE_ONLY>
__global__ void __launch_bounds__(256) blend_backward_t_kernel(BlendArgs a, int ntiles,
                                                               const float* __restrict__ final_T,
                                                               const uint32_t* __restrict__ n_contrib,
                                                               const float* __restrict__ dL_dcolor,
                                                               const float* __restrict__ dL_ddepth,
                                                               float* __restrict__ grad_acc) {
    __shared__ __attribute__((aligned(16))) float s_fac[4][2][BT_SLOTS][WAVE];
    __shared__ BtMetaRec s_meta[4][BT_SLOTS];
    __shared__ __attribute__((aligned(16))) float s_pix[4][POSE_ONLY ? 1 : 4][16][4];
    const int wave = __builtin_amdgcn_readfirstlane((int)(threadIdx.x >> 6)), lane = threadIdx.x & 63;
    const int tile = (int)blockIdx.x;
    if (tile >= ntiles) return;
    const int tx = tile % a.gx, ty = tile / a.gx;
    const uint2 range = a.ranges[tile];
    if (range.y <= range.x) return;
    const size_t HW = (size_t)a.H * a.W;
    const float bg0 = a.bg[0], bg1 = a.bg[1], bg2 = a.bg[2];

    const int qx0i = tx * TILE + (wave & 1) * SUB, qy0i = ty * TILE + (wave >> 1) * SUB;
    const int pxi = qx0i + (lane & 7), pyi = qy0i + (lane >> 3);
    const bool inside = pxi < a.W && pyi < a.H;
    const size_t pix = (size_t)pyi * a.W + pxi;
    const float pxf = (float)pxi, pyf = (float)pyi, qx0 = (float)qx0i, qy0 = (float)qy0i;
    const float T_final = inside ? final_T[pix] : 0.f;
    const uint32_t last = inside ? n_contrib[pix] : 0u;
    const float g0 = inside ? dL_dcolor[pix] : 0.f;
    const float g1 = inside ? dL_dcolor[HW + pix] : 0.f;
    const float g2 = inside ? dL_dcolor[2 * HW + pix] : 0.f;
    const float gd = inside ? dL_ddepth[pix] : 0.f;
    const float bgT = -T_final * (bg0 * g0 + bg1 * g1 + bg2 * g2);
    float T = T_final, Bk = 0.f;
    const uint32_t maxc = (uint32_t)__builtin_amdgcn_readfirstlane((int)wave_max_u32(last));
    if (maxc == 0) return;
    const uint32_t end = range.x + maxc;

    const int q = lane & 15;
    const int fxi = qx0i + 4 * (q & 1), fyi = qy0i + (q >> 1);
    if (lane < 16) {
#pragma unroll
        for (int i = 0; i < 4; ++i) {
            const bool in_i = (fxi + i) < a.W && fyi < a.H;
            const size_t px_i = (size_t)fyi * a.W + fxi + i;
            if (!POSE_ONLY) {
                s_pix[wave][0][q][i] = in_i ? dL_dcolor[px_i] : 0.f;
                s_pix[wave][1][q][i] = in_i ? dL_dcolor[HW + px_i] : 0.f;
                s_pix[wave][2][q][i] = in_i ? dL_dcolor[2 * HW + px_i] : 0.f;
            }
            s_pix[wave][POSE_ONLY ? 0 : 3][q][i] = in_i ? dL_ddepth[px_i] : 0.f;
        }
    }
    const int slot = POSE_ONLY ? bt_slot6(q) : bt_slot10(q);
    const uint32_t slot_bytes = slot < 0 ? 0u : (uint32_t)slot * 4u;
    const unsigned long long m_out = __builtin_amdgcn_ballot_w64(slot >= 0);
    const unsigned long long m_q0 = __builtin_amdgcn_ballot_w64((q & 3) == 0), m_q1 = __builtin_amdgcn_ballot_w64((q & 3) == 1);
    float* const fhl = &s_fac[wave][0][0][lane];
    BtMetaRec* const fmeta = &s_meta[wave][0];
    const BtLane bl{&s_fac[wave][0][0][0], &s_pix[wave][0][0][0], fmeta, lane, qx0, qy0, slot_bytes, m_out, m_q0, m_q1, grad_acc};
    int k = 0;

    uint32_t gid_n = 0;
    float4 box_n = make_float4(0.f, 0.f, -1.f, -1.f), ell_n = make_float4(0.f, 0.f, 0.f, 0.f);
    auto prefetch = [&](int b) {
        gid_n = 0;
        box_n = make_float4(0.f, 0.f, -1.f, -1.f);
        const uint32_t i = range.x + (uint32_t)b * WAVE + lane;
        if (b >= 0 && i < end) {
            gid_n = a.point_list[i];
            box_n = a.rec[(size_t)gid_n * 4];
            ell_n = a.rec[(size_t)gid_n * 4 + 3];
        }
    };
    prefetch((int)((maxc - 1) / WAVE));
    for (int b = (int)((maxc - 1) / WAVE); b >= 0; --b) {
        const uint32_t gid_l = gid_n;
        const float4 c = box_n, el = ell_n;
        prefetch(b - 1);
        const unsigned long long alive = __builtin_amdgcn_ballot_w64(last >= (uint32_t)b * WAVE + 1u);
        unsigned long long mask = __builtin_amdgcn_ballot_w64(quadrant_hit(c, el, qx0, qy0, alive));
        const uint32_t k_first = (uint32_t)b * WAVE + 1u;
        auto apply = [&](const Rec& g, int j, float power, float G, float alpha) {
            const bool act = (k_first + (uint32_t)j <= last) && !(power > 0.f) && !(alpha < 1.0f / 255.0f);
            if (__builtin_amdgcn_ballot_w64(act) == 0ull) return;
            const float a_eff = act ? alpha : 0.f;
            const float inv = __builtin_amdgcn_rcpf(1.f - a_eff);
            const float Tn = T * inv;
            const float qq = __builtin_fmaf(g.z, gd, __builtin_fmaf(g.b, g2, __builtin_fmaf(g.g, g1, g.r * g0)));
            const float diff = qq - Bk;
            const float dL_dalpha = diff * Tn + bgT * inv;
            Bk = Bk + a_eff * diff;
            T = Tn;
            const float w = a_eff * Tn;
            const float h = act ? G * dL_dalpha : 0.f;
            fhl[k * WAVE] = h;
            fhl[(BT_SLOTS + k) * WAVE] = w;
            if (__builtin_amdgcn_inverse_ballot_w64(1ull << j)) fmeta[k] = BtMetaRec{c.x, c.y, gid_l};
            if (++k == BT_SLOTS) {
                bt_flush<POSE_ONLY>(bl, BT_SLOTS);
                k = 0;
            }
        };
        while (mask) {
            const int j = 63 - __builtin_clzll(mask);
            mask &= ~(1ull << j);
            const Rec g = fetch(a, bcast(gid_l, j));
            const float dx = g.px - pxf, dy = g.py - pyf;
            const float power = dx * (g.ca * dx + g.cb * dy) + (g.cc * dy) * dy;
            const float G = __builtin_amdgcn_exp2f(power);
            apply(g, j, power, G, fminf(0.99f, g.op * G));
        }
    }
    if (k) bt_flush<POSE_ONLY>(bl, k);
}

typedef float v2f __attribute__((ext_vector_type(2)));
typedef float v3f __attribute__((ext_vector_type(3)));
typedef float v8f __attribute__((ext_vector_type(8)));
template <bool POSE_ONLY>
__global__ void __launch_bounds__(256) blend_backward_s_kernel(BlendArgs a, int ntiles,
                                                               const float* __restrict__ final_T,
                                                               const uint32_t* __restrict__ n_contrib,
                                                               const float* __restrict__ dL_dcolor,
                                                               const float* __restrict__ dL_ddepth,
                                                               float* __restrict__ grad_acc) {
    struct WaveLds { float h[BT_SLOTS][BS_STRIDE / 4]; float pad[(BS_W_OFF - BT_SLOTS * BS_STRIDE) / 4]; float w[BT_SLOTS][BS_STRIDE / 4];
                     BtMetaRec meta[BT_SLOTS][BS_STRIDE / 16]; };
    static_assert(sizeof(WaveLds) == BS_META_OFF + BT_SLOTS * BS_STRIDE, "layout");
    __shared__ __attribute__((aligned(16))) WaveLds s_w[MGS_WG_WAVES];
    __shared__ __attribute__((aligned(16))) float s_pix[MGS_WG_WAVES][POSE_ONLY ? 1 : 4][16][4];
    MGS_TILE_WAVE(ntiles, tile, wave, ws)
    const int lane = threadIdx.x & 63;
    const int tx = tile % a.gx, ty = tile / a.gx;
    const uint2 range = a.ranges[tile];
    if (range.y <= range.x) return;
    const size_t HW = (size_t)a.H * a.W;
    const float bg0 = a.bg[0], bg1 = a.bg[1], bg2 = a.bg[2];

    const int qx0i = tx * TILE + (wave & 1) * SUB, qy0i = ty * TILE + (wave >> 1) * SUB;
    const int pxi = qx0i + (lane & 7), pyi = qy0i + (lane >> 3);
    const bool inside = pxi < a.W && pyi < a.H;
    const size_t pix = (size_t)pyi * a.W + pxi;
    const float pxf = (float)pxi, pyf = (float)pyi;
    const float T_final = inside ? final_T[pix] : 0.f;
    const uint32_t last = inside ? n_contrib[pix] : 0u;
    const float g0 = inside ? dL_dcolor[pix] : 0.f;
    const float g1 = inside ? dL_dcolor[HW + pix] : 0.f;
    const float g2 = inside ? dL_dcolor[2 * HW + pix] : 0.f;
    const float gd = inside ? dL_ddepth[pix] : 0.f;
    const float bgT = -T_final * (bg0 * g0 + bg1 * g1 + bg2 * g2);
    float T = T_final, Bk = 0.f;
    const uint32_t maxc = (uint32_t)__builtin_amdgcn_readfirstlane((int)wave_max_u32(last));
    if (maxc == 0) return;
    const uint32_t end = range.x + maxc;
#ifdef BS_TRACE
    unsigned long long tr0;
    uint32_t tr_n = 0;
    BS_STAMP(tr0);
#endif

    const int q = lane & 15;
    const int fxi = qx0i + 4 * (q & 1), fyi = qy0i + (q >> 1);
    if (lane < 16) {
#pragma unroll
        for (int i = 0; i < 4; ++i) {
            const bool in_i = (fxi + i) < a.W && fyi < a.H;
            const size_t px_i = (size_t)fyi * a.W + fxi + i;
            if (!POSE_ONLY) {
                s_pix[ws][0][q][i] = in_i ? dL_dcolor[px_i] : 0.f;
                s_pix[ws][1][q][i] = in_i ? dL_dcolor[HW + px_i] : 0.f;
                s_pix[ws][2][q][i] = in_i ? dL_dcolor[2 * HW + px_i] : 0.f;
            }
            s_pix[ws][POSE_ONLY ? 0 : 3][q][i] = in_i ? dL_ddepth[px_i] : 0.f;
        }
    }
    const int slot = POSE_ONLY ? bt_slot6(q) : bt_slot10(q);
    const uint32_t slot_bytes = slot < 0 ? 0u : (uint32_t)slot * 4u;
    const unsigned long long m_out = __builtin_amdgcn_ballot_w64(slot >= 0);
    const unsigned long long m_q0 = __builtin_amdgcn_ballot_w64((q & 3) == 0), m_q1 = __builtin_amdgcn_ballot_w64((q & 3) == 1);
    const BtLane bl{&s_w[ws].h[0][0], &s_pix[ws][0][0][0], &s_w[ws].meta[0][0], lane, 0.f, 0.f, slot_bytes, m_out, m_q0, m_q1, grad_acc, qx0i, qy0i};
    const uint32_t wbase = (uint32_t)__builtin_amdgcn_readfirstlane((int)(uint32_t)(uintptr_t)&s_w[ws]);
    const const_float_p recs = MGS_CONST(reinterpret_cast<const float*>(a.rec));
    uint32_t koff = 0;
    float zero = 0.f;
    asm volatile("" : "+v"(zero));

    uint32_t gid_n = 0;
    float4 box_n = make_float4(0.f, 0.f, -1.f, -1.f), ell_n = make_float4(0.f, 0.f, 0.f, 0.f);
    auto prefetch = [&](int b) {
        gid_n = 0;
        box_n = make_float4(0.f, 0.f, -1.f, -1.f);
        const uint32_t i = range.x + (uint32_t)b * WAVE + (uint32_t)(63 - lane);
        if (b >= 0 && i < end) {
            gid_n = a.point_list[i];
            box_n = a.rec[(size_t)gid_n * 4];
            ell_n = a.rec[(size_t)gid_n * 4 + 3];
        }
    };
    prefetch((int)((maxc - 1) / WAVE));
    for (int b = (int)((maxc - 1) / WAVE); b >= 0; --b) {
        const float4 c = box_n, el = ell_n;
        v3f meta = {c.x, c.y, __uint_as_float(gid_n << 6)};
        prefetch(b - 1);
        const unsigned long long alive = __builtin_amdgcn_ballot_w64(last >= (uint32_t)b * WAVE + 1u);
        int qxs = qx0i, qys = qy0i;
        asm volatile("" : "+s"(qxs), "+s"(qys));
        unsigned long long mask = __builtin_amdgcn_ballot_w64(quadrant_hit(c, el, (float)qxs, (float)qys, alive));
        const int thr = 63 + (int)((uint32_t)b * WAVE + 1u) - (int)last;
#define BS_POP(J, R0, R1)                                                                                                    \
        asm volatile("s_ff1_i32_b64 %0, %1\n\ts_bitset0_b64 %1, %0" : "=&s"(J), "+s"(mask));                                 \
        {                                                                                                                    \
            const uint32_t goff = (uint32_t)__builtin_amdgcn_readlane((int)__float_as_uint(meta[2]), J);                     \
            asm volatile("s_load_dwordx2 %0, %2, %3\n\ts_load_dwordx8 %1, %2, %3 offset:0x10"                                \
                         : "=&s"(R0), "=&s"(R1) : "s"(recs), "s"(goff) : "memory");                                          \
        }
        auto evaluate = [&](const v2f r0, const v8f r1, const int j) {
                float dx, dy, t1, t2, G, al, inv, qq;
                uint32_t adv, sa, tmp;
                asm volatile(
                    "v_sub_f32_e32 %[dx], %[px], %[pxf]\n\t"
                    "v_sub_f32_e32 %[dy], %[py], %[pyf]\n\t"
                    "v_mul_f32_e32 %[t1], %[cb], %[dy]\n\t"
                    "v_mul_f32_e32 %[t2], %[cc], %[dy]\n\t"
                    "v_fmac_f32_e32 %[t1], %[ca], %[dx]\n\t"
                    "v_mul_f32_e32 %[t2], %[dy], %[t2]\n\t"
                    "v_fmac_f32_e32 %[t2], %[dx], %[t1]\n\t"
                    "v_exp_f32_e32 %[G], %[t2]\n\t"
                    "s_add_u32 %[tmp], %[wbase], %[koff]\n\t"
                    "v_lshl_add_u32 %[sa], %[lane], 2, %[tmp]\n\t"
                    "ds_write2st64_b32 %[sa], %[zero], %[zero] offset1:5\n\t"
                    "v_cmpx_ge_i32_e32 vcc, %[j], %[thr]\n\t"
                    "v_cmpx_nlt_f32_e32 vcc, 0, %[t2]\n\t"
                    "v_mul_f32_e32 %[al], %[op], %[G]\n\t"
                    "v_min_f32_e32 %[al], 0x3f7d70a4, %[al]\n\t"
                    "v_cmpx_ngt_f32_e32 vcc, %[amin], %[al]\n\t"
                    "v_sub_f32_e32 %[inv], 1.0, %[al]\n\t"
                    "v_rcp_f32_e32 %[inv], %[inv]\n\t"
                    "v_mul_f32_e32 %[qq], %[cr], %[g0]\n\t"
                    "v_fmac_f32_e32 %[qq], %[cg], %[g1]\n\t"
                    "v_fmac_f32_e32 %[qq], %[cb2], %[g2]\n\t"
                    "v_fmac_f32_e32 %[qq], %[cz], %[gd]\n\t"
                    "v_mul_f32_e32 %[T], %[T], %[inv]\n\t"
                    "v_sub_f32_e32 %[qq], %[qq], %[Bk]\n\t"
                    "v_mul_f32_e32 %[dx], %[T], %[qq]\n\t"
                    "v_fmac_f32_e32 %[dx], %[bgT], %[inv]\n\t"
                    "v_mul_f32_e32 %[dx], %[G], %[dx]\n\t"
                    "v_mul_f32_e32 %[dy], %[al], %[T]\n\t"
                    "v_fmac_f32_e32 %[Bk], %[al], %[qq]\n\t"
                    "ds_write2st64_b32 %[sa], %[dx], %[dy] offset1:5\n\t"
                    "s_cmp_lg_u64 exec, 0\n\t"
                    "s_cselect_b32 %[adv], 272, 0\n\t"
                    "s_lshl_b64 exec, 1, %[j]\n\t"
                    "v_mov_b32_e32 %[sa], %[tmp]\n\t"
                    "ds_write_b96 %[sa], %[meta] offset:2368\n\t"
                    "s_mov_b64 exec, -1\n\t"
                    : [dx] "=&v"(dx), [dy] "=&v"(dy), [t1] "=&v"(t1), [t2] "=&v"(t2), [G] "=&v"(G), [al] "=&v"(al), [inv] "=&v"(inv),
                      [qq] "=&v"(qq), [sa] "=&v"(sa), [T] "+v"(T), [Bk] "+v"(Bk), [adv] "=&s"(adv), [tmp] "=&s"(tmp)
                    : [px] "s"(r0[0]), [py] "s"(r0[1]), [ca] "s"(r1[0]), [cb] "s"(r1[1]), [cc] "s"(r1[2]), [op] "s"(r1[3]),
                      [cr] "s"(r1[4]), [cg] "s"(r1[5]), [cb2] "s"(r1[6]), [cz] "s"(r1[7]), [pxf] "v"(pxf), [pyf] "v"(pyf), [thr] "v"(thr),
                      [j] "s"(j), [g0] "v"(g0), [g1] "v"(g1), [g2] "v"(g2), [gd] "v"(gd), [bgT] "v"(bgT), [lane] "v"(lane), [zero] "v"(zero),
                      [koff] "s"(koff), [wbase] "s"(wbase), [meta] "v"(meta), [amin] "s"(1.0f / 255.0f)
                    : "vcc", "scc", "memory");
                koff += adv;
            if (koff == BT_SLOTS * BS_STRIDE) {
                bt_flush<POSE_ONLY, true>(bl, BT_SLOTS);
                koff = 0;
            }
        };
#ifdef BS_TRACE
        tr_n += (uint32_t)__popcll(mask);
#endif
        if (mask) {
            int jA, jB = 0;
            v2f a0, b0;
            v8f a1, b1;
            BS_POP(jA, a0, a1)
            for (;;) {
                asm volatile("s_waitcnt lgkmcnt(0)" : "+s"(a0), "+s"(a1) : : "memory");
                const bool moreB = mask != 0ull;
                if (moreB) { BS_POP(jB, b0, b1) }
                evaluate(a0, a1, jA);
                if (!moreB) break;
                asm volatile("s_waitcnt lgkmcnt(0)" : "+s"(b0), "+s"(b1) : : "memory");
                const bool moreA = mask != 0ull;
                if (moreA) { BS_POP(jA, a0, a1) }
                evaluate(b0, b1, jB);
                if (!moreA) break;
            }
        }
#undef BS_POP
    }
    if (koff) bt_flush<POSE_ONLY, true>(bl, (int)(koff >> 8));
#ifdef BS_TRACE
    if (a.trace) {
        unsigned long long tr1;
        BS_STAMP(tr1);
        const unsigned hw = __builtin_amdgcn_s_getreg((31 << 11) | 4), xcc = __builtin_amdgcn_s_getreg((31 << 11) | 20);
        if (lane == 0) {
            unsigned long long* o = a.trace + ((size_t)tile * 4 + wave) * 4;
            o[0] = tr0; o[1] = tr1; o[2] = (unsigned long long)hw | ((unsigned long long)xcc << 32); o[3] = tr_n;
        }
    }
#endif
}

__global__ void __launch_bounds__(256) blend_backward_stats_kernel(BlendArgs a, int ntiles,
                                                                   const uint32_t* __restrict__ n_contrib,
                                                                   unsigned long long* __restrict__ stats) {
    const int wave = threadIdx.x >> 6, lane = threadIdx.x & 63;
    const int tile = (int)blockIdx.x;
    if (tile >= ntiles) return;
    const int tx = tile % a.gx, ty = tile / a.gx;
    const uint2 range = a.ranges[tile];
    if (range.y <= range.x) return;
    const int qx0i = tx * TILE + (wave & 1) * SUB, qy0i = ty * TILE + (wave >> 1) * SUB;
    const int pxi = qx0i + (lane & 7), pyi = qy0i + (lane >> 3);
    const bool inside = pxi < a.W && pyi < a.H;
    const float pxf = (float)pxi, pyf = (float)pyi, qx0 = (float)qx0i, qy0 = (float)qy0i;
    const uint32_t last = inside ? n_contrib[(size_t)pyi * a.W + pxi] : 0u;
    const uint32_t maxc = wave_max_u32(last);
    if (maxc == 0) return;
    const uint32_t end = range.x + maxc;
    unsigned long long c[8] = {0, 0, 0, 0, 0, 0, 0, 0};
    for (int b = (int)((maxc - 1) / WAVE); b >= 0; --b) {
        const uint32_t i = range.x + (uint32_t)b * WAVE + lane;
        uint32_t gid_l = 0;
        float4 box = make_float4(0.f, 0.f, -1.f, -1.f), el = make_float4(0.f, 0.f, 0.f, 0.f);
        if (i < end) {
            gid_l = a.point_list[i];
            box = a.rec[(size_t)gid_l * 4];
            el = a.rec[(size_t)gid_l * 4 + 3];
        }
        const unsigned long long alive = __builtin_amdgcn_ballot_w64(last >= (uint32_t)b * WAVE + 1u);
        unsigned long long mask = __builtin_amdgcn_ballot_w64(quadrant_hit(box, el, qx0, qy0, alive));
        c[0] += 1;
        c[1] += __popcll(mask);
        while (mask) {
            const int j = 63 - __builtin_clzll(mask);
            mask &= ~(1ull << j);
            const uint32_t k = (uint32_t)b * WAVE + (uint32_t)j + 1u;
            const Rec g = fetch(a, bcast(gid_l, j));
            const float dx = g.px - pxf, dy = g.py - pyf;
            const float power = dx * (g.ca * dx + g.cb * dy) + (g.cc * dy) * dy;
            const float alpha = fminf(0.99f, g.op * __builtin_amdgcn_exp2f(power));
            const bool geo = !(power > 0.f) && !(alpha < 1.0f / 255.0f);
            const unsigned long long act = __builtin_amdgcn_ballot_w64(geo && k <= last);
            const int n = __popcll(act);
            if (n == 0) {
                if (__builtin_amdgcn_ballot_w64(geo) != 0ull) c[4] += 1;
                continue;
            }
            c[2] += 1;
            c[3] += n;
            c[5] += n <= 2;
            c[6] += n <= 4;
            c[7] += n <= 8;
        }
    }
    if (lane < 8) {
        unsigned long long v = c[0];
#pragma unroll
        for (int q = 1; q < 8; ++q) v = lane == q ? c[q] : v;
        atomicAdd(stats + lane, v);
    }
}

__device__ __forceinline__ bool rect_hit(const float4 c, const float4 n, float qx0, float qy0, int ox, int oy, int w, int h,
                                         unsigned long long alive) {
    if (c.z < 0.f) return false;
    const float x0q = qx0 - 0.05f - c.x, y0q = qy0 - 0.05f - c.y;
    const float x0 = x0q + (float)ox, x1 = qx0 + (float)(ox + w - 1) + 0.05f - c.x;
    const float y0 = y0q + (float)oy, y1 = qy0 + (float)(oy + h - 1) + 0.05f - c.y;
    if (!((c.z >= x0) && (-c.z <= x1) && (c.w >= y0) && (-c.w <= y1))) return false;
    {
        const int ix0 = (int)fminf(8.f, fmaxf(0.f, ceilf(-x0q - c.z - 0.06f))), ix1 = (int)fminf(7.f, fmaxf(-1.f, floorf(-x0q + c.z + 0.06f)));
        const int iy0 = (int)fminf(8.f, fmaxf(0.f, ceilf(-y0q - c.w - 0.06f))), iy1 = (int)fminf(7.f, fmaxf(-1.f, floorf(-y0q + c.w + 0.06f)));
        if (ix0 > ix1 || iy0 > iy1) return false;
        const unsigned long long cols = (unsigned long long)((0xFFu >> (7 - ix1)) & (0xFFu << ix0) & 0xFFu) * 0x0101010101010101ull;
        const unsigned long long rows = (~0ull >> (8 * (7 - iy1))) & (~0ull << (8 * iy0));
        const unsigned long long gcols = (unsigned long long)(((1u << w) - 1u) << ox) * 0x0101010101010101ull;
        const unsigned long long grows = ((h >= 8 ? ~0ull : ((1ull << (8 * h)) - 1ull)) << (8 * oy));
        if ((cols & rows & gcols & grows & alive) == 0ull) return false;
    }
    if (x0 <= 0.f && x1 >= 0.f && y0 <= 0.f && y1 >= 0.f) return true;
    if (!(n.x > 0.f) || !(n.z > 0.f)) return true;
    const float rby = -n.y * __builtin_amdgcn_rcpf(n.z), rbx = -n.y * __builtin_amdgcn_rcpf(n.x);
    auto edge_x = [&](float xe) { const float t = fminf(y1, fmaxf(y0, rby * xe)); return n.x * xe * xe + 2.f * n.y * xe * t + n.z * t * t; };
    auto edge_y = [&](float ye) { const float t = fminf(x1, fmaxf(x0, rbx * ye)); return n.x * t * t + 2.f * n.y * t * ye + n.z * ye * ye; };
    return fminf(fminf(edge_x(x0), edge_x(x1)), fminf(edge_y(y0), edge_y(y1))) <= 1.02f;
}
__global__ void __launch_bounds__(256) blend_group_stats_kernel(BlendArgs a, int ntiles, const uint32_t* __restrict__ n_contrib,
                                                                unsigned long long* __restrict__ stats) {
    const int wave = threadIdx.x >> 6, lane = threadIdx.x & 63;
    const int tile = (int)blockIdx.x;
    if (tile >= ntiles) return;
    const int tx = tile % a.gx, ty = tile / a.gx;
    const uint2 range = a.ranges[tile];
    if (range.y <= range.x) return;
    const int qx0i = tx * TILE + (wave & 1) * SUB, qy0i = ty * TILE + (wave >> 1) * SUB;
    const int pxi = qx0i + (lane & 7), pyi = qy0i + (lane >> 3);
    const bool inside = pxi < a.W && pyi < a.H;
    const float qx0 = (float)qx0i, qy0 = (float)qy0i;
    const uint32_t last = inside ? n_contrib[(size_t)pyi * a.W + pxi] : 0u;
    const uint32_t maxc = wave_max_u32(last);
    if (maxc == 0) return;
    const uint32_t end = range.x + maxc;
    constexpr int ND = 5;
    constexpr int NG[ND] = {2, 2, 4, 4, 8}, GW[ND] = {8, 4, 4, 8, 4}, GH[ND] = {4, 8, 4, 2, 2}, GX[ND] = {1, 2, 2, 1, 2};
    unsigned long long trips_step[ND] = {0, 0, 0, 0, 0}, rows[ND] = {0, 0, 0, 0, 0};
    uint32_t walk[ND][8];
#pragma unroll
    for (int d = 0; d < ND; ++d)
#pragma unroll
        for (int g = 0; g < 8; ++g) walk[d][g] = 0;
    for (int b = (int)((maxc - 1) / WAVE); b >= 0; --b) {
        const uint32_t i = range.x + (uint32_t)b * WAVE + lane;
        float4 box = make_float4(0.f, 0.f, -1.f, -1.f), el = make_float4(0.f, 0.f, 0.f, 0.f);
        if (i < end) {
            const uint32_t gid_l = a.point_list[i];
            box = a.rec[(size_t)gid_l * 4];
            el = a.rec[(size_t)gid_l * 4 + 3];
        }
        const unsigned long long alive = __builtin_amdgcn_ballot_w64(last >= (uint32_t)b * WAVE + 1u);
#pragma unroll
        for (int d = 0; d < ND; ++d) {
            int mx = 0, sum = 0;
#pragma unroll
            for (int g = 0; g < NG[d]; ++g) {
                const int ox = (g % GX[d]) * GW[d], oy = (g / GX[d]) * GH[d];
                const int n = __popcll(__builtin_amdgcn_ballot_w64(rect_hit(box, el, qx0, qy0, ox, oy, GW[d], GH[d], alive)));
                mx = max(mx, n);
                sum += n;
                walk[d][g] += (uint32_t)n;
            }
            trips_step[d] += mx;
            rows[d] += sum;
        }
    }
    if (lane == 0) {
#pragma unroll
        for (int d = 0; d < ND; ++d) {
            uint32_t mx = 0;
#pragma unroll
            for (int g = 0; g < NG[d]; ++g) mx = max(mx, walk[d][g]);
            atomicAdd(stats + 8 + 3 * d + 0, trips_step[d]);
            atomicAdd(stats + 8 + 3 * d + 1, rows[d]);
            atomicAdd(stats + 8 + 3 * d + 2, (unsigned long long)mx);
        }
    }
}

int launch_blend_backward_stats(const mgs_camera& cam, const GeometryState& g, const BinningState& b,
                                const ImageState& img, unsigned long long* stats, hipStream_t s) {
    const BlendArgs a = make_args(cam, g, b, img);
    const int ntiles = a.gx * tiles_y(a.H);
    if (ntiles == 0) return 0;
    hipLaunchKernelGGL(blend_backward_stats_kernel, dim3(ntiles), dim3(256), 0, s, a, ntiles, img.n_contrib, stats);
    hipLaunchKernelGGL(blend_group_stats_kernel, dim3(ntiles), dim3(256), 0, s, a, ntiles, img.n_contrib, stats);
    MGS_HIP(hipGetLastError());
    return 0;
}

int g_opt_blend_lds_pad_fwd = 0, g_opt_blend_lds_pad_bwd = 0;
int g_opt_blend_bwd_transposed = 2;
int launch_blend_backward(const mgs_camera& cam, const GeometryState& g, const BinningState& b,
                          const ImageState& img, const float* dL_dcolor, const float* dL_ddepth, float* grad_acc,
                          bool pose_only, hipStream_t s) {
    BlendArgs a = make_args(cam, g, b, img);
#ifdef BS_TRACE
    a.trace = g_trace_bwd;
#endif
    const int ntiles = a.gx * tiles_y(a.H);
    if (ntiles == 0) return 0;
    if (g_opt_blend_bwd_transposed == 2) {
        const dim3 grid(ntiles), block(256);
        if (pose_only)
            hipLaunchKernelGGL((blend_backward_s_kernel<true>), grid, block, (size_t)g_opt_blend_lds_pad_bwd, s, a, ntiles, img.final_T,
                               img.n_contrib, dL_dcolor, dL_ddepth, grad_acc);
        else
            hipLaunchKernelGGL((blend_backward_s_kernel<false>), grid, block, (size_t)g_opt_blend_lds_pad_bwd, s, a, ntiles, img.final_T,
                               img.n_contrib, dL_dcolor, dL_ddepth, grad_acc);
    } else if (g_opt_blend_bwd_transposed != 0) {
        if (pose_only)
            hipLaunchKernelGGL((blend_backward_t_kernel<true>), dim3(ntiles), dim3(256), 0, s, a, ntiles, img.final_T,
                               img.n_contrib, dL_dcolor, dL_ddepth, grad_acc);
        else
            hipLaunchKernelGGL((blend_backward_t_kernel<false>), dim3(ntiles), dim3(256), 0, s, a, ntiles, img.final_T,
                               img.n_contrib, dL_dcolor, dL_ddepth, grad_acc);
    } else if (pose_only)
        hipLaunchKernelGGL((blend_backward_kernel<true>), dim3(ntiles), dim3(256), 0, s, a, ntiles, img.final_T,
                           img.n_contrib, dL_dcolor, dL_ddepth, grad_acc);
    else
        hipLaunchKernelGGL((blend_backward_kernel<false>), dim3(ntiles), dim3(256), 0, s, a, ntiles, img.final_T,
                           img.n_contrib, dL_dcolor, dL_ddepth, grad_acc);
    MGS_HIP(hipGetLastError());
    return 0;
}

__global__ void __launch_bounds__(256) valu_ceiling_kernel(float* out, int iters, float seed) {
    float a0 = seed + threadIdx.x, a1 = a0 + 1, a2 = a0 + 2, a3 = a0 + 3, a4 = a0 + 4, a5 = a0 + 5, a6 = a0 + 6, a7 = a0 + 7;
    const float c = 1.0001f, d = 0.0001f;
    for (int i = 0; i < iters; ++i) {
        a0 = __builtin_fmaf(a0, c, d); a1 = __builtin_fmaf(a1, c, d); a2 = __builtin_fmaf(a2, c, d); a3 = __builtin_fmaf(a3, c, d);
        a4 = __builtin_fmaf(a4, c, d); a5 = __builtin_fmaf(a5, c, d); a6 = __builtin_fmaf(a6, c, d); a7 = __builtin_fmaf(a7, c, d);
    }
    out[blockIdx.x * 256 + threadIdx.x] = ((a0 + a1) + (a2 + a3)) + ((a4 + a5) + (a6 + a7));
}
int launch_valu_ceiling(float* out, int iters, hipStream_t s) {
    hipLaunchKernelGGL(valu_ceiling_kernel, dim3(MGS_VALU_CEILING_BLOCKS), dim3(256), 0, s, out, iters, 1.0f);
    MGS_HIP(hipGetLastError());
    return 0;
}

}

#ifdef BS_TRACE
extern "C" int mgs_trace_set_blend_buffers(void* fwd, void* bwd) {
    mgs::g_trace_fwd = (unsigned long long*)fwd;
    mgs::g_trace_bwd = (unsigned long long*)bwd;
    return 0;
}
#endif
```

### monogs_amd/csrc/common.h

```cpp
#pragma once

#include <hip/hip_runtime.h>
#include <stdint.h>
#include <stddef.h>

#include "../../include/monogs_raster.h"

namespace mgs {

constexpr int TILE = MGS_TILE;
constexpr int WAVE = 64;
constexpr int SUB = 8;
constexpr int REC_FLOATS = 16;
constexpr int GRAD_FLOATS = 16;

enum : int {
    R_X = 0, R_Y = 1, R_EX = 2, R_EY = 3,
    R_CA = 4, R_CB = 5, R_CC = 6, R_OPAC = 7,
    R_R = 8, R_G = 9, R_B = 10, R_DEPTH = 11,
    R_NA = 12, R_NB = 13, R_NC = 14, R_RADIUS = 15
};
enum : int {
    G_SX = 0, G_SY = 1, G_SXX = 2, G_SXY = 3, G_SYY = 4, G_SH = 5,
    G_DR = 6, G_DG = 7, G_DB = 8, G_DDEPTH = 9
};

inline size_t align_up(size_t v, size_t a) { return (v + a - 1) / a * a; }

#if defined(__HIP_DEVICE_COMPILE__)
typedef const float __attribute__((address_space(4))) * const_float_p;
#define MGS_CONST(p) ((mgs::const_float_p)(p))
#else
typedef const float* const_float_p;
#define MGS_CONST(p) (p)
#endif

__device__ __forceinline__ uint32_t wave_incl_scan_dpp(uint32_t v) {
#define MGS_DPP_ADD(ctrl, row_mask) v += (uint32_t)__builtin_amdgcn_update_dpp(0, (int)v, ctrl, row_mask, 0xf, false)
    MGS_DPP_ADD(0x111, 0xf);
    MGS_DPP_ADD(0x112, 0xf);
    MGS_DPP_ADD(0x114, 0xf);
    MGS_DPP_ADD(0x118, 0xf);
    MGS_DPP_ADD(0x142, 0xa);
    MGS_DPP_ADD(0x143, 0xc);
#undef MGS_DPP_ADD
    return v;
}

__global__ static void zero_fill_kernel(uint32_t* __restrict__ p, size_t n_words, int vec) {
    const size_t i0 = (size_t)blockIdx.x * blockDim.x + threadIdx.x, stride = (size_t)gridDim.x * blockDim.x;
    if (vec) {
        uint4* q = reinterpret_cast<uint4*>(p);
        const size_t nv = n_words / 4;
        for (size_t i = i0; i < nv; i += stride) q[i] = make_uint4(0u, 0u, 0u, 0u);
        for (size_t i = nv * 4 + i0; i < n_words; i += stride) p[i] = 0u;
    } else {
        for (size_t i = i0; i < n_words; i += stride) p[i] = 0u;
    }
}
__device__ __forceinline__ void grid_zero(uint32_t* __restrict__ p, size_t n_words, size_t threads, int block) {
    const size_t i0 = (size_t)blockIdx.x * block + threadIdx.x, stride = threads;
    uint4* q = reinterpret_cast<uint4*>(p);
    const size_t nv = n_words / 4;
    for (size_t i = i0; i < nv; i += stride) q[i] = make_uint4(0u, 0u, 0u, 0u);
    for (size_t i = nv * 4 + i0; i < n_words; i += stride) p[i] = 0u;
}
__global__ static void zero_fill2_kernel(uint32_t* __restrict__ p, size_t n_words, uint32_t* __restrict__ p2, int n2) {
    grid_zero(p, n_words, (size_t)gridDim.x * 256, 256);
    if (blockIdx.x == 0 && (int)threadIdx.x < n2) p2[threadIdx.x] = 0u;
}
static inline hipError_t zero_fill2(void* ptr, size_t bytes, void* ptr2, size_t bytes2, hipStream_t s) {
    const size_t n_words = bytes / 4;
    size_t blocks = (n_words / 4 + 255) / 256;
    blocks = blocks < 1 ? 1 : (blocks > 4096 ? 4096 : blocks);
    hipLaunchKernelGGL(zero_fill2_kernel, dim3((unsigned)blocks), dim3(256), 0, s, (uint32_t*)ptr, n_words,
                       (uint32_t*)ptr2, ptr2 ? (int)(bytes2 / 4) : 0);
    return hipGetLastError();
}
static inline hipError_t zero_fill(void* ptr, size_t bytes, hipStream_t s) {
    if (bytes == 0) return hipSuccess;
    const size_t n_words = bytes / 4;
    const int vec = ((size_t)ptr % 16 == 0) ? 1 : 0;
    const size_t items = vec ? (n_words + 3) / 4 : n_words;
    size_t blocks = (items + 255) / 256;
    if (blocks > 4096) blocks = 4096;
    hipLaunchKernelGGL(zero_fill_kernel, dim3((unsigned)blocks), dim3(256), 0, s, (uint32_t*)ptr, n_words, vec);
    return hipGetLastError();
}

struct GeometryState {
    float* rec;
    uint32_t* depth_key;
    uint32_t* depth_alt;
    uint32_t* iota;
    uint32_t* iota_alt;
    uint32_t* perm;
    uint32_t* point_offsets;
    uint32_t* scan_blocks;
    uint8_t* clamped;
    uint2* rect;
    uint2* rect_sorted;
    uint64_t* scan_status;
    uint32_t* tile_hist;
    void* sort_temp;
    size_t sort_temp_bytes;
    char* end;
    static size_t bytes(int P);
    static GeometryState carve(void* base, int P);
};
constexpr int SCAN_SMALL_MAX_BLOCKS = 64;

struct ImageState {
    float* final_T;
    uint32_t* n_contrib;
    uint2* ranges;
    static size_t bytes(int W, int H);
    static ImageState carve(void* base, int W, int H);
};

struct BinningState {
    uint32_t* keys_a;
    uint32_t* vals_a;
    uint32_t* keys_b;
    uint32_t* vals_b;
    uint32_t* keys_sorted;
    uint32_t* vals_sorted;
    void* sort_temp;
    size_t sort_temp_bytes;
    uint32_t* count;
    static size_t bytes(uint64_t R, int W, int H);
    static BinningState carve(void* base, uint64_t R, int W, int H);
};

constexpr int SCAN_ITEMS = 2048;
inline int scan_nblocks(int P) { return (P + SCAN_ITEMS - 1) / SCAN_ITEMS; }

inline int tiles_x(int W) { return (W + TILE - 1) / TILE; }
inline int tiles_y(int H) { return (H + TILE - 1) / TILE; }
inline int tile_bits(int W, int H) {
    uint32_t n = (uint32_t)(tiles_x(W) * tiles_y(H));
    int b = 0;
    while ((1u << b) < n && b < 31) ++b;
    return b == 0 ? 1 : b;
}

constexpr uint32_t DEPTH_KEY_SUB = 0x3E4CCCCDu;
constexpr uint32_t DEPTH_KEY_NARROW = (1u << 27) - 1u;
__host__ __device__ inline int tile_depth_lo_bits(int tb) { return tb > 5 ? tb - 5 : 0; }
int binning_path(int P, int W, int H);

void set_error(const char* fmt, ...);
#define MGS_HIP(expr)                                                                     \
    do {                                                                                  \
        hipError_t _e = (expr);                                                           \
        if (_e != hipSuccess) {                                                           \
            mgs::set_error("%s failed: %s (%s:%d)", #expr, hipGetErrorString(_e), __FILE__, __LINE__); \
            return 2;                                                                     \
        }                                                                                 \
    } while (0)

struct StageTimer;

int launch_preprocess_forward(const mgs_camera& cam, int P, const float* means3D, const float* shs,
                              const float* colors_precomp, const float* opacities, const float* scales,
                              const float* rotations, const float* cov3D_precomp,
                              const GeometryState& g, int32_t* radii, float* prepare_grad_acc, hipStream_t s);
constexpr int TAU_SLOTS = 256;
inline float* backward_grad_acc(void* scratch) { return (float*)align_up((size_t)scratch, 256); }
inline float* backward_tau_part(void* scratch, int P) { return backward_grad_acc(scratch) + (size_t)P * GRAD_FLOATS; }
inline float* backward_tau_out(void* scratch, int P) { return backward_tau_part(scratch, P) + (size_t)TAU_SLOTS * 16; }
int launch_scan(const GeometryState& g, int P, hipStream_t s, bool exclusive, const uint2* rects);
bool depth_chain_is_small(int P);
int launch_depth_chain_small(const GeometryState& g, int P, hipStream_t s);
int launch_duplicate(const mgs_camera& cam, int P, const GeometryState& g, const BinningState& b, uint64_t r_cap,
                     int32_t* n_touched, const ImageState& img, uint64_t sort_n, int sort_bits, uint32_t* count,
                     uint32_t* overflow, hipStream_t s, bool per_tile);
size_t sort_temp_bytes(uint64_t n, int bits);
size_t radix_temp_bytes(uint64_t n, int bits);
size_t radix_depth_temp_bytes(uint64_t n);
bool radix_result_in_b(int bits);
constexpr int RADIX_ERROR_WORDS = 4;
const uint32_t* radix_error_flag(void* temp, uint64_t n, int bits);
const uint32_t* radix_depth_error_flag(void* temp, uint64_t n);
__device__ __forceinline__ uint32_t radix_failed(const uint32_t* __restrict__ e) { return (e[0] | e[1]) | (e[2] | e[3]); }
void radix_zero_region(void* temp, uint64_t n, int bits, uint32_t** ptr, size_t* words);
void radix_depth_zero_region(void* temp, uint64_t n, uint32_t** ptr, size_t* words, bool header_only = false);
int radix_sort_pairs(uint32_t* ka, uint32_t* va, uint32_t* kb, uint32_t* vb, uint64_t n, int bits, void* temp,
                     hipStream_t s, const uint32_t* n_dev = nullptr, bool temp_zeroed = false,
                     const uint2* aux_in = nullptr, uint2* aux_out = nullptr,
                     const uint32_t* ext_hist = nullptr,
                     bool aux_empty_for_ones = false,
                     bool exclusive = false,
                     uint2* ranges = nullptr,
                     int key_shift = 0);
bool radix_wants_hist(uint64_t n);
bool radix_depth_payload(uint64_t n);
int radix_sort_depth(uint32_t* keys, uint32_t* key_b, uint32_t* val_a, uint32_t* val_b, void* rect, bool payload,
                     uint32_t* perm, uint2* rect_sorted, uint64_t n, void* temp, hipStream_t s, bool temp_zeroed,
                     bool exclusive = false);
inline bool depth_sort_payload(int P, int W, int H) { return radix_depth_payload((uint64_t)P) && tiles_x(W) <= 255 && tiles_y(H) <= 255; }
int launch_depth_sort(const GeometryState& g, int P, bool payload, hipStream_t s, bool exclusive = false);
int launch_sort(const GeometryState& g, const BinningState& b, uint64_t R, int bits, hipStream_t s,
                const uint32_t* n_dev = nullptr, bool exclusive = false, uint2* ranges = nullptr, bool per_tile = false);
struct TileSortArgs {
    uint32_t* keys;
    uint32_t* vals;
    uint32_t* keys_alt;
    uint32_t* vals_alt;
    const uint32_t* depth_key;
    const uint32_t* n_dev;
    uint32_t n_cap;
    int tb;
};
TileSortArgs tile_sort_args(const mgs_camera& cam, const GeometryState& g, const BinningState& b, uint64_t R,
                            const uint32_t* n_dev);
int launch_tile_depth_sort(const mgs_camera& cam, const TileSortArgs& ts, const ImageState& img, const uint32_t* sort_err,
                           hipStream_t s);
int set_radix_spin_limit(uint32_t limit);
extern int g_opt_radix_ballot_rank, g_opt_radix_scanned, g_opt_radix_xcd_band, g_opt_radix_tile_items, g_opt_knn_grid_min, g_opt_scan_small, g_opt_dup_slot_major, g_opt_blend_bwd_transposed, g_opt_blend_lds_pad_fwd, g_opt_blend_lds_pad_bwd, g_opt_depth_small;
int launch_blend_forward(const mgs_camera& cam, const GeometryState& g, const BinningState& b,
                         const ImageState& img, float* out_color, float* out_depth, float* out_opacity,
                         int32_t* n_touched, const uint32_t* sort_err, uint32_t* status, const TileSortArgs* tile_sort,
                         hipStream_t s);
int launch_blend_backward(const mgs_camera& cam, const GeometryState& g, const BinningState& b,
                          const ImageState& img, const float* dL_dcolor, const float* dL_ddepth,
                          float* grad_acc, bool pose_only, hipStream_t s);
int launch_blend_backward_stats(const mgs_camera& cam, const GeometryState& g, const BinningState& b,
                                const ImageState& img, unsigned long long* stats, hipStream_t s);
int launch_valu_ceiling(float* out, int iters, hipStream_t s);
struct GeomBackwardArgs {
    const float *means3D, *shs, *colors_precomp, *opacities, *scales, *rotations, *cov3D_precomp;
    const int32_t* radii;
    const float* grad_acc;
    float *dL_dmeans2D, *dL_dcolors, *dL_dopacity, *dL_dmeans3D, *dL_dcov3D, *dL_dsh, *dL_dscales,
        *dL_drotations, *dL_dtau;
    float* tau_part;
};
constexpr int TAU_DIRECT_MAX_BLOCKS = 256;
int launch_geom_backward(const mgs_camera& cam, int P, const GeometryState& g, const GeomBackwardArgs& a,
                         hipStream_t s);
int launch_mark_visible(int P, const float* means3D, const float* viewmatrix, uint8_t* visible, hipStream_t s);
size_t knn_scratch_bytes(int P);
int launch_knn(int P, const float* points, float* out, void* scratch, hipStream_t s);

}
```

### monogs_amd/rasterizer.py

```python
from __future__ import annotations

import contextlib
import ctypes as C
from typing import NamedTuple, Optional

import torch
import torch.nn as nn

from . import _lib


class GaussianRasterizationSettings(NamedTuple):
    image_height: int
    image_width: int
    tanfovx: float
    tanfovy: float
    bg: torch.Tensor
    scale_modifier: float
    viewmatrix: torch.Tensor
    projmatrix: torch.Tensor
    projmatrix_raw: torch.Tensor
    sh_degree: int
    campos: torch.Tensor
    prefiltered: bool
    debug: bool


_sync_free = {"enabled": False, "headroom": 1.5}
HINTS_MAX, PENDING_MAX = 64, 1024


class _State:
    capacity_hint: dict = {}
    pending: list = []
    graph: list = []
    exact_pending = None
    exact_other: list = []
    exact_failed = 0


_capacity_hint = _State.capacity_hint
_pending_overflow = _State.pending
_graph_overflow = _State.graph


def _remember_hint(key, R):
    h = _State.capacity_hint
    if key not in h and len(h) >= HINTS_MAX:
        h.pop(next(iter(h)))
    h[key] = R


def set_sync_free(enabled: bool, headroom: float = 1.5):
    _sync_free["enabled"], _sync_free["headroom"] = bool(enabled), float(headroom)


def sync_free_enabled() -> bool:
    return bool(_sync_free["enabled"])


_call_flags = {"exclusive": False}


@contextlib.contextmanager
def exclusive_device(on: bool = True):
    prev, _call_flags["exclusive"] = _call_flags["exclusive"], bool(on)
    try:
        yield
    finally:
        _call_flags["exclusive"] = prev


STATUS_CAPACITY_OVERFLOW, STATUS_DEPTH_SORT_TIMEOUT, STATUS_TILE_SORT_TIMEOUT = 1, 2, 4


def _raise_sort_failure(bits):
    which = [n for b, n in ((STATUS_DEPTH_SORT_TIMEOUT, "depth sort"), (STATUS_TILE_SORT_TIMEOUT, "tile sort")) if bits & b]
    raise RuntimeError(f"rasteriser: a look-back spin of the {' and the '.join(which)} timed out; "
                       "the renders since the last check are invalid")


def _drain_exact_other(n: int) -> None:
    old, _State.exact_other = _State.exact_other[:n], _State.exact_other[n:]
    for d in {e[2] for e in old}:
        torch.cuda.synchronize(d)
    for e in old:
        _State.exact_failed |= int(e[1].item()) & (STATUS_DEPTH_SORT_TIMEOUT | STATUS_TILE_SORT_TIMEOUT)


def check_overflow() -> bool:
    hit, sort_fail = False, _State.exact_failed
    _State.exact_failed = 0
    exact = _State.exact_other + ([_State.exact_pending] if _State.exact_pending is not None else [])
    _State.exact_pending = None
    _State.exact_other = []
    for d in {e[2] for e in exact} | {f.device.index for _, f in _State.pending + _State.graph}:
        torch.cuda.synchronize(d)
    todo = _State.pending + _State.graph + [(e[0], e[1]) for e in exact]
    for key, flag in todo:
        v = int(flag.item())
        if v & STATUS_CAPACITY_OVERFLOW:
            hit = True
            _remember_hint(key, max(2 * _State.capacity_hint.get(key, 1), 1024))
        sort_fail |= v & (STATUS_DEPTH_SORT_TIMEOUT | STATUS_TILE_SORT_TIMEOUT)
    _State.pending.clear()
    if sort_fail:
        _raise_sort_failure(sort_fail)
    return hit


def clear_graph_flags():
    _State.graph.clear()


_timing_sink: Optional[list] = None


@contextlib.contextmanager
def collect_timing():
    global _timing_sink
    prev, _timing_sink = _timing_sink, []
    try:
        yield _timing_sink
    finally:
        _timing_sink = prev


def _ptr(t: Optional[torch.Tensor]):
    return None if t is None else t.data_ptr()


def _al(n: int) -> int:
    return (int(n) + 255) // 256 * 256


def _f32(t: torch.Tensor, name: str) -> torch.Tensor:
    if not t.is_cuda:
        raise RuntimeError(f"{name} must be a CUDA/HIP tensor (got device {t.device}); "
                           "the rasteriser has no CPU path")
    if t.dtype != torch.float32:
        raise RuntimeError(f"{name} must be float32 (got {t.dtype})")
    return t.contiguous()


def _camera(rs: GaussianRasterizationSettings, sh_coeffs: int, keep: list, scale_dim: int = 3) -> _lib.MgsCamera:
    cam = _lib.MgsCamera()
    cam.scale_dim = int(scale_dim)
    cam.flags = 1 if _call_flags["exclusive"] else 0
    cam.image_height, cam.image_width = int(rs.image_height), int(rs.image_width)
    cam.tanfovx, cam.tanfovy = float(rs.tanfovx), float(rs.tanfovy)
    cam.scale_modifier = float(rs.scale_modifier)
    cam.sh_degree, cam.sh_coeffs = int(rs.sh_degree), int(sh_coeffs)
    for field in ("bg", "viewmatrix", "projmatrix", "projmatrix_raw", "campos"):
        t = _f32(getattr(rs, field).detach(), f"raster_settings.{field}")
        keep.append(t)
        setattr(cam, field, t.data_ptr())
    return cam


_raw_stream = getattr(torch._C, "_cuda_getCurrentRawStream", None)


class _device_guard:
    __slots__ = ("idx", "prev")

    def __init__(self, dev):
        idx = getattr(dev, "index", dev)
        self.idx = torch._C._cuda_getDevice() if idx is None else int(idx)

    def __enter__(self):
        self.prev = torch._C._cuda_getDevice()
        if self.prev != self.idx:
            torch._C._cuda_setDevice(self.idx)
        return self

    def __exit__(self, *exc):
        if self.prev != self.idx:
            torch._C._cuda_setDevice(self.prev)
        return False


def _stream():
    if _raw_stream is not None:
        return _raw_stream(torch._C._cuda_getDevice())
    return torch.cuda.current_stream().cuda_stream


class _RasterizeGaussians(torch.autograd.Function):
    @staticmethod
    def forward(ctx, means3D, means2D, sh, colors_precomp, opacities, scales, rotations, cov3Ds_precomp,
                theta, rho, raster_settings):
        lib = _lib.load()
        rs = raster_settings
        means3D = _f32(means3D.detach(), "means3D")
        P = means3D.shape[0]
        dev = means3D.device
        opt = lambda t, n: _f32(t.detach(), n) if (t is not None and t.numel() > 0) else None
        sh_ = opt(sh, "shs")
        col_ = opt(colors_precomp, "colors_precomp")
        opac_ = _f32(opacities.detach(), "opacities")
        sc_ = opt(scales, "scales")
        rot_ = opt(rotations, "rotations")
        cov_ = opt(cov3Ds_precomp, "cov3D_precomp")
        M = 0 if sh_ is None else int(sh_.shape[1])
        H, W = int(rs.image_height), int(rs.image_width)

        with _device_guard(dev):
            keep = []
            scale_dim = int(sc_.shape[1]) if sc_ is not None else 3
            if scale_dim not in (1, 3):
                raise Exception("scales must be [P,3] (or [P,1] for an isotropic map)")
            cam = _camera(rs, M, keep, scale_dim)
            timing = _lib.MgsTiming() if _timing_sink is not None else None
            tref = C.byref(timing) if timing is not None else None
            u8 = dict(dtype=torch.uint8, device=dev)
            want_bwd = P > 0 and any(ctx.needs_input_grad)
            n_geom, n_img = _al(lib.mgs_geometry_bytes(P)), _al(lib.mgs_image_bytes(W, H))
            n_bwd = _al(lib.mgs_backward_bytes(P)) if want_bwd else 0
            arena = torch.empty(n_geom + n_img + n_bwd + 256, **u8)
            base = arena.data_ptr()
            off0 = (-base) % 256
            geom_p, img_p = base + off0, base + off0 + n_geom
            o_r = off0 + n_geom + n_img
            ri = torch.empty(2, P, dtype=torch.int32, device=dev)
            radii, n_touched = ri[0], ri[1]
            ctx.scratch = arena[o_r:o_r + n_bwd] if want_bwd else None
            bwd_p = base + o_r if want_bwd else None
            ctx.scratch_used = False
            out5 = torch.empty(5, H, W, dtype=torch.float32, device=dev)
            color, depth, opacity = out5[0:3], out5[3:4], out5[4:5]
            status = torch.empty(1, dtype=torch.int32, device=dev) if P > 0 else None
            key = (P, W, H)
            capturing = torch.cuda.is_current_stream_capturing()
            hint = _State.capacity_hint.get(key)
            if capturing and hint is None:
                raise RuntimeError("graph capture needs a capacity hint: run one eager forward with the same "
                                   "(P, W, H) first")
            if _State.exact_failed and not capturing:
                bits, _State.exact_failed = _State.exact_failed, 0
                _raise_sort_failure(bits)
            if (capturing or _sync_free["enabled"]) and hint is not None and P > 0:
                R = max(int(hint * _sync_free["headroom"]) + 4096, 4096)
                binning = torch.empty(lib.mgs_binning_bytes(R, W, H), **u8)
                _lib.check(lib.mgs_forward_capacity(
                    C.byref(cam), P, _ptr(means3D), _ptr(sh_), _ptr(col_), _ptr(opac_), _ptr(sc_), _ptr(rot_), _ptr(cov_),
                    geom_p, radii.data_ptr(), bwd_p, R, binning.data_ptr(), img_p, color.data_ptr(), depth.data_ptr(),
                    opacity.data_ptr(), n_touched.data_ptr(), status.data_ptr(), tref, _stream()), "mgs_forward_capacity")
                (_State.graph if capturing else _State.pending).append((key, status))
                if len(_State.pending) > PENDING_MAX:
                    del _State.pending[:PENDING_MAX // 2]
                ctx.overflow = status
            else:
                num_rendered, prev_bits = C.c_uint64(0), C.c_uint32(0)
                prev = _State.exact_pending
                here = (torch._C._cuda_getDevice(), _stream())
                if prev is not None and (prev[2], prev[3]) != here:
                    _State.exact_other.append(prev)
                    if len(_State.exact_other) > PENDING_MAX:
                        _drain_exact_other(PENDING_MAX // 2)
                    prev = None
                _lib.check(lib.mgs_forward_preprocess(
                    C.byref(cam), P, _ptr(means3D), _ptr(sh_), _ptr(col_), _ptr(opac_), _ptr(sc_), _ptr(rot_),
                    _ptr(cov_), geom_p, radii.data_ptr(), bwd_p, C.byref(num_rendered),
                    prev[1].data_ptr() if prev is not None else None, C.byref(prev_bits) if prev is not None else None,
                    tref, _stream()), "mgs_forward_preprocess")
                _State.exact_pending = None
                if prev_bits.value & (STATUS_DEPTH_SORT_TIMEOUT | STATUS_TILE_SORT_TIMEOUT):
                    _raise_sort_failure(prev_bits.value)
                R = int(num_rendered.value)
                _remember_hint(key, R)
                binning = torch.empty(lib.mgs_binning_bytes(R, W, H), **u8)
                _lib.check(lib.mgs_forward_render(
                    C.byref(cam), P, R, geom_p, binning.data_ptr(), img_p, color.data_ptr(),
                    depth.data_ptr(), opacity.data_ptr(), n_touched.data_ptr(), _ptr(status), tref, _stream()),
                    "mgs_forward_render")
                if status is not None:
                    _State.exact_pending = (key, status, here[0], here[1])
                ctx.overflow = None
            if rs.debug:
                check_overflow()
            if timing is not None:
                d = timing.as_dict()
                d.update(kind="forward", num_rendered=R, P=P)
                _timing_sink.append(d)

        ctx.cam, ctx.keep = cam, keep
        ctx.geom_off, ctx.img_off = off0, off0 + n_geom
        ctx.raster_settings = rs
        ctx.num_rendered = R
        ctx.sh_coeffs = M
        ctx.scale_dim = scale_dim
        ctx.has = (sh_ is not None, col_ is not None, sc_ is not None, cov_ is not None,
                   theta is not None, rho is not None)
        dummy = torch.empty(0, device=dev)
        ctx.save_for_backward(means3D, sh_ if sh_ is not None else dummy, col_ if col_ is not None else dummy,
                              opac_, sc_ if sc_ is not None else dummy, rot_ if rot_ is not None else dummy,
                              cov_ if cov_ is not None else dummy, radii, arena, binning)
        ctx.mark_non_differentiable(radii, n_touched)
        ctx.set_materialize_grads(False)
        return color, radii, depth, opacity, n_touched

    @staticmethod
    def backward(ctx, grad_color, grad_radii, grad_depth, grad_opacity, grad_n_touched):
        lib = _lib.load()
        rs = ctx.raster_settings
        means3D, sh_, col_, opac_, sc_, rot_, cov_, radii, arena, binning = ctx.saved_tensors
        geom_p, img_p = arena.data_ptr() + ctx.geom_off, arena.data_ptr() + ctx.img_off
        has_sh, has_col, has_sr, has_cov, has_theta, has_rho = ctx.has
        P = means3D.shape[0]
        dev = means3D.device
        H, W = int(rs.image_height), int(rs.image_width)
        need = ctx.needs_input_grad

        with _device_guard(dev):
            cam = ctx.cam
            f32 = dict(dtype=torch.float32, device=dev)
            g_color = _f32(grad_color, "grad_color") if grad_color is not None else torch.zeros(3, H, W, **f32)
            g_depth = _f32(grad_depth, "grad_depth") if grad_depth is not None else torch.zeros(1, H, W, **f32)
            out = lambda cond, *shape: torch.empty(*shape, **f32) if cond else None
            d_means2D = out(need[1], P, 3)
            d_sh = out(need[2] and has_sh, P, max(ctx.sh_coeffs, 1), 3)
            d_cov = out(need[7] and has_cov, P, 6)
            widths = [3 if need[0] else 0, 3 if (need[3] and has_col) else 0, 1 if need[4] else 0,
                      ctx.scale_dim if (need[5] and has_sr) else 0, 4 if (need[6] and has_sr) else 0]
            flat = torch.empty(P * sum(widths), **f32) if sum(widths) else None
            views, o = [], 0
            for w in widths:
                views.append(flat[o:o + P * w].view(P, w) if w else None)
                o += P * w
            d_means3D, d_col, d_opac, d_scales, d_rot = views
            want_tau = (need[8] and has_theta) or (need[9] and has_rho)
            prepared = ctx.scratch is not None and not ctx.scratch_used
            ctx.scratch_used = True
            scratch = ctx.scratch if prepared else torch.empty(lib.mgs_backward_bytes(P), dtype=torch.uint8, device=dev)
            if want_tau and prepared:
                off = int(lib.mgs_backward_tau(scratch.data_ptr(), P)) - scratch.data_ptr()
                d_tau = scratch[off:off + 24].view(torch.float32)
            else:
                d_tau = torch.empty(6, **f32) if want_tau else None
            timing = _lib.MgsTiming() if _timing_sink is not None else None
            tref = C.byref(timing) if timing is not None else None
            _lib.check(lib.mgs_backward(
                C.byref(cam), P, ctx.num_rendered,
                _ptr(means3D), _ptr(sh_) if has_sh else None, _ptr(col_) if has_col else None, _ptr(opac_),
                _ptr(sc_) if has_sr else None, _ptr(rot_) if has_sr else None, _ptr(cov_) if has_cov else None,
                radii.data_ptr(), geom_p, binning.data_ptr(), img_p,
                g_color.data_ptr(), g_depth.data_ptr(),
                _ptr(d_means2D), _ptr(d_col), _ptr(d_opac), _ptr(d_means3D), _ptr(d_cov), _ptr(d_sh),
                _ptr(d_scales), _ptr(d_rot), _ptr(d_tau), scratch.data_ptr(), 1 if prepared else 0, tref, _stream()),
                "mgs_backward")
            if timing is not None:
                d = timing.as_dict()
                d.update(kind="backward", num_rendered=ctx.num_rendered, P=P)
                _timing_sink.append(d)
        d_theta = d_tau[3:] if (d_tau is not None and need[8] and has_theta) else None
        d_rho = d_tau[:3] if (d_tau is not None and need[9] and has_rho) else None
        return (d_means3D, d_means2D, d_sh, d_col, d_opac, d_scales, d_rot, d_cov, d_theta, d_rho, None)


def debug_blend_stats(color: torch.Tensor) -> dict:
    fn = color.grad_fn
    if fn is None or not hasattr(fn, "raster_settings"):
        raise RuntimeError("debug_blend_stats needs the colour image of a differentiable rasteriser forward")
    lib = _lib.load()
    means3D, _, _, _, _, _, _, _, arena, binning = fn.saved_tensors
    cam = fn.cam
    out = torch.zeros(24, dtype=torch.int64, device=means3D.device)
    with _device_guard(means3D.device):
        _lib.check(lib.mgs_debug_blend_stats(C.byref(cam), means3D.shape[0], fn.num_rendered,
                                             arena.data_ptr() + fn.geom_off, binning.data_ptr(),
                                             arena.data_ptr() + fn.img_off, out.data_ptr(), _stream()),
                   "mgs_debug_blend_stats")
    v = out.tolist()
    groups = {}
    for d, name in enumerate(("halves_8x4", "halves_4x8", "blocks_4x4", "strips_8x2", "blocks_4x2")):
        groups[name] = dict(trips_paired_per_step=v[8 + 3 * d], rows=v[9 + 3 * d], trips_own_lists=v[10 + 3 * d])
    return dict(steps=v[0], survivors=v[1], active_survivors=v[2], active_pairs=v[3], inactive_by_depth_order=v[4],
                active_le2=v[5], active_le4=v[6], active_le8=v[7], group_streams=groups)


def rasterize_gaussians(means3D, means2D, sh, colors_precomp, opacities, scales, rotations, cov3Ds_precomp,
                        theta, rho, raster_settings):
    return _RasterizeGaussians.apply(means3D, means2D, sh, colors_precomp, opacities, scales, rotations,
                                     cov3Ds_precomp, theta, rho, raster_settings)


class GaussianRasterizer(nn.Module):
    def __init__(self, raster_settings: GaussianRasterizationSettings):
        super().__init__()
        self.raster_settings = raster_settings

    def markVisible(self, positions: torch.Tensor) -> torch.Tensor:
        lib = _lib.load()
        rs = self.raster_settings
        with torch.no_grad():
            pos = _f32(positions, "positions")
            P = pos.shape[0]
            vis = torch.zeros(P, dtype=torch.uint8, device=pos.device)
            with _device_guard(pos.device):
                vm = _f32(rs.viewmatrix, "viewmatrix")
                pm = _f32(rs.projmatrix, "projmatrix")
                _lib.check(lib.mgs_mark_visible(P, pos.data_ptr(), vm.data_ptr(), pm.data_ptr(), vis.data_ptr(),
                                                _stream()), "mgs_mark_visible")
        return vis.bool()

    def forward(self, means3D, means2D, opacities, shs=None, colors_precomp=None, scales=None, rotations=None,
                cov3D_precomp=None, theta=None, rho=None):
        rs = self.raster_settings
        if (shs is None and colors_precomp is None) or (shs is not None and colors_precomp is not None):
            raise Exception("Please provide excatly one of either SHs or precomputed colors!")
        if ((scales is None or rotations is None) and cov3D_precomp is None) or \
                ((scales is not None or rotations is not None) and cov3D_precomp is not None):
            raise Exception("Please provide exactly one of either scale/rotation pair or precomputed 3D covariance!")
        return rasterize_gaussians(means3D, means2D, shs, colors_precomp, opacities, scales, rotations,
                                   cov3D_precomp, theta, rho, rs)
```

Before: 2878 Mpix/s.

## Split blend backward per tile into front and back walks using forward outputs

The backward blend kernel can now cut each tile's per-pixel Gaussian list at a split point and process the two halves in separate workgroups. The front half walks forward from T=1, seeded with the forward output colour and depth, while the back half walks backward from final_T as before. This doubles the grid and shortens the serial chain per wave when tiles are heavy (num_rendered >= 128 per tile), aiming to fix load imbalance and the long serial latency. It requires passing out_color/out_depth into backward, tracked through a weakref plus version check, and adds more gradient atomics and some accumulated float-rounding differences.

```diff
diff --git a/include/monogs_raster.h b/include/monogs_raster.h
--- a/include/monogs_raster.h
+++ b/include/monogs_raster.h
@@ -8,7 +8,7 @@
 extern "C" {
 #endif
 
-#define MGS_ABI_VERSION 10
+#define MGS_ABI_VERSION 11
 #define MGS_TILE 16
 
 typedef struct mgs_camera {
@@ -103,6 +103,7 @@
                  const float* cov3D_precomp, const int32_t* radii,
                  const void* geometry, const void* binning, const void* image,
                  const float* dL_dcolor, const float* dL_ddepth,
+                 const float* out_color, const float* out_depth,
                  float* dL_dmeans2D,
                  float* dL_dcolors,
                  float* dL_dopacity,
@@ -118,6 +119,8 @@
 int mgs_debug_valu_ceiling(float* out, int32_t iters, void* stream);
 
 int mgs_debug_set_blend_events(void* fwd_start, void* fwd_end, void* bwd_start, void* bwd_end);
+
+int mgs_debug_last_backward_split(void);
 
 #define MGS_BLEND_STATS_WORDS 24
 int mgs_debug_blend_stats(const mgs_camera* cam, int32_t P, uint64_t num_rendered, const void* geometry,
diff --git a/monogs_amd/_lib.py b/monogs_amd/_lib.py
--- a/monogs_amd/_lib.py
+++ b/monogs_amd/_lib.py
@@ -5,7 +5,7 @@
 
 _HERE = os.path.dirname(os.path.abspath(__file__))
 LIB_PATH = os.environ.get("MGS_LIB_PATH") or os.path.join(_HERE, "lib", "libmonogs_raster.so")
-ABI_VERSION = 10
+ABI_VERSION = 11
 
 c_float_p = C.c_void_p
 
@@ -51,12 +51,13 @@
     "mgs_forward_render_capacity": (C.c_int, [C.POINTER(MgsCamera), C.c_int32, C.c_uint64] + [C.c_void_p] * 8
                                     + [C.POINTER(MgsTiming), C.c_void_p]),
     "mgs_backward": (C.c_int, [C.POINTER(MgsCamera), C.c_int32, C.c_uint64] + [C.c_void_p] * 7
-                     + [C.c_void_p] * 4 + [C.c_void_p] * 2 + [C.c_void_p] * 9
+                     + [C.c_void_p] * 4 + [C.c_void_p] * 4 + [C.c_void_p] * 9
                      + [C.c_void_p, C.c_int32, C.POINTER(MgsTiming), C.c_void_p]),
     "mgs_backward_tau": (C.c_void_p, [C.c_void_p, C.c_int32]),
     "mgs_debug_blend_stats": (C.c_int, [C.POINTER(MgsCamera), C.c_int32, C.c_uint64] + [C.c_void_p] * 5),
     "mgs_debug_valu_ceiling": (C.c_int, [C.c_void_p, C.c_int32, C.c_void_p]),
     "mgs_debug_set_blend_events": (C.c_int, [C.c_void_p] * 4),
+    "mgs_debug_last_backward_split": (C.c_int, []),
     "mgs_mark_visible": (C.c_int, [C.c_int32, C.c_void_p, C.c_void_p, C.c_void_p, C.c_void_p, C.c_void_p]),
     "mgs_loss_scratch_bytes": (C.c_size_t, []),
     "mgs_loss_forward": (C.c_int, [C.c_int32] * 4 + [C.c_float] + [C.c_void_p] * 9 + [C.c_void_p, C.c_void_p, C.c_void_p]),
diff --git a/monogs_amd/csrc/api.hip b/monogs_amd/csrc/api.hip
--- a/monogs_amd/csrc/api.hip
+++ b/monogs_amd/csrc/api.hip
@@ -297,8 +297,8 @@
 int mgs_backward(const mgs_camera* cam, int32_t P, uint64_t R, const float* means3D, const float* shs,
                  const float* colors_precomp, const float* opacities, const float* scales, const float* rotations,
                  const float* cov3D_precomp, const int32_t* radii, const void* geometry, const void* binning,
-                 const void* image, const float* dL_dcolor, const float* dL_ddepth, float* dL_dmeans2D,
-                 float* dL_dcolors, float* dL_dopacity, float* dL_dmeans3D, float* dL_dcov3D, float* dL_dsh,
+                 const void* image, const float* dL_dcolor, const float* dL_ddepth, const float* out_color,
+                 const float* out_depth, float* dL_dmeans2D, float* dL_dcolors, float* dL_dopacity, float* dL_dmeans3D, float* dL_dcov3D, float* dL_dsh,
                  float* dL_dscales, float* dL_drotations, float* dL_dtau, void* backward_scratch,
                  int32_t scratch_prepared, mgs_timing* timing, void* stream) {
     if (check_cam(cam)) return 1;
@@ -334,7 +334,7 @@
     if (R > 0) {
         const bool pose_only = !dL_dcolors && !dL_dopacity && !dL_dsh && !shs;
         if (g_dbg_bwd_events[0]) MGS_HIP(hipEventRecord(g_dbg_bwd_events[0], s));
-        if (int rc = launch_blend_backward(*cam, g, b, img, dL_dcolor, dL_ddepth, grad_acc, pose_only, s)) return rc;
+        if (int rc = launch_blend_backward(*cam, g, b, img, dL_dcolor, dL_ddepth, out_color, out_depth, grad_acc, pose_only, R, s)) return rc;
         if (g_dbg_bwd_events[1]) MGS_HIP(hipEventRecord(g_dbg_bwd_events[1], s));
     }
     tm.mark();
@@ -374,6 +374,8 @@
     return launch_valu_ceiling(out, iters, (hipStream_t)stream);
 }
 
+int mgs_debug_last_backward_split(void) { return g_dbg_last_bwd_split; }
+
 int mgs_debug_set_radix_spin_limit(uint32_t limit) { return set_radix_spin_limit(limit); }
 
 int mgs_debug_set_blend_events(void* fwd_start, void* fwd_end, void* bwd_start, void* bwd_end) {
@@ -417,7 +419,14 @@
     if (name && !strcmp(name, "radix_xcd_band")) { g_opt_radix_xcd_band = (int)value; return 0; }
     if (name && !strcmp(name, "debug_sort_exclusive")) { g_opt_debug_sort_exclusive = (int)value; return 0; }
     if (name && !strcmp(name, "dup_slot_major")) { g_opt_dup_slot_major = (int)value; return 0; }
-    if (name && !strcmp(name, "blend_bwd_transposed")) { g_opt_blend_bwd_transposed = (int)value; return 0; }
+    if (name && !strcmp(name, "blend_bwd_transposed")) {
+        g_opt_blend_bwd_transposed = value < 0 ? 2 : (int)value;
+        g_opt_blend_bwd_transposed_set = value >= 0;
+        return 0;
+    }
+    if (name && !strcmp(name, "blend_bwd_split")) { g_opt_blend_bwd_split = value < 0 ? -1 : (int)value; return 0; }
+    if (name && !strcmp(name, "blend_bwd_split_min")) { g_opt_blend_bwd_split_min = value < 0 ? 4 : (int)value; return 0; }
+    if (name && !strcmp(name, "blend_bwd_split_frac")) { g_opt_blend_bwd_split_frac = value < 0 ? 32 : (int)value; return 0; }
     if (name && !strcmp(name, "scan_small")) { g_opt_scan_small = (int)value; return 0; }
     if (name && !strcmp(name, "depth_small")) { g_opt_depth_small = (int)value; return 0; }
     if (name && !strcmp(name, "tile_sort_fused")) { g_opt_tile_sort_fused = value < 0 ? 1 : (int)value; return 0; }
diff --git a/monogs_amd/csrc/blend.hip b/monogs_amd/csrc/blend.hip
--- a/monogs_amd/csrc/blend.hip
+++ b/monogs_amd/csrc/blend.hip
@@ -10,6 +10,7 @@
 #ifdef BS_TRACE
 static unsigned long long* g_trace_fwd = nullptr;
 static unsigned long long* g_trace_bwd = nullptr;
+static unsigned long long g_trace_bwd_records = 0;
 #define BS_STAMP(v) asm volatile("s_memrealtime %0\n\ts_waitcnt lgkmcnt(0)" : "=s"(v) :: "memory")
 #endif
 
@@ -743,42 +744,57 @@
 typedef float v2f __attribute__((ext_vector_type(2)));
 typedef float v3f __attribute__((ext_vector_type(3)));
 typedef float v8f __attribute__((ext_vector_type(8)));
-template <bool POSE_ONLY>
-__global__ void __launch_bounds__(256) blend_backward_s_kernel(BlendArgs a, int ntiles,
-                                                               const float* __restrict__ final_T,
-                                                               const uint32_t* __restrict__ n_contrib,
-                                                               const float* __restrict__ dL_dcolor,
-                                                               const float* __restrict__ dL_ddepth,
-                                                               float* __restrict__ grad_acc) {
-    struct WaveLds { float h[BT_SLOTS][BS_STRIDE / 4]; float pad[(BS_W_OFF - BT_SLOTS * BS_STRIDE) / 4]; float w[BT_SLOTS][BS_STRIDE / 4];
-                     BtMetaRec meta[BT_SLOTS][BS_STRIDE / 16]; };
-    static_assert(sizeof(WaveLds) == BS_META_OFF + BT_SLOTS * BS_STRIDE, "layout");
-    __shared__ __attribute__((aligned(16))) WaveLds s_w[MGS_WG_WAVES];
-    __shared__ __attribute__((aligned(16))) float s_pix[MGS_WG_WAVES][POSE_ONLY ? 1 : 4][16][4];
-    MGS_TILE_WAVE(ntiles, tile, wave, ws)
+constexpr int BS_SPLIT_MIN = 4, BS_SPLIT_FRAC = 32;
+struct BsSplit { int min_steps, frac256; };
+__device__ __forceinline__ uint32_t bs_split_point(uint32_t maxc, BsSplit sp) {
+    const uint32_t steps = (maxc + WAVE - 1) / WAVE;
+    if (steps < 2u || steps < (uint32_t)sp.min_steps) return 0u;
+    const uint32_t f = (maxc * (uint32_t)sp.frac256 / 256u + WAVE / 2) / WAVE;
+    return min(max(f, 1u), steps - 1u) * WAVE;
+}
+struct BsWaveLds { float h[BT_SLOTS][BS_STRIDE / 4]; float pad[(BS_W_OFF - BT_SLOTS * BS_STRIDE) / 4]; float w[BT_SLOTS][BS_STRIDE / 4];
+                   BtMetaRec meta[BT_SLOTS][BS_STRIDE / 16]; };
+static_assert(sizeof(BsWaveLds) == BS_META_OFF + BT_SLOTS * BS_STRIDE, "layout");
+template <bool POSE_ONLY, int DIR>
+__device__ __forceinline__ void bs_walk(const BlendArgs& a, const int tile, const int job, const int wave, BsWaveLds* const s_w_ws, float* const s_pix_ws,
+                                        const float* __restrict__ final_T, const uint32_t* __restrict__ n_contrib,
+                                        const float* __restrict__ dL_dcolor, const float* __restrict__ dL_ddepth,
+                                        const float* __restrict__ out_color, const float* __restrict__ out_depth,
+                                        float* __restrict__ grad_acc, const BsSplit sp) {
+    constexpr bool FRONT = DIR == 2;
     const int lane = threadIdx.x & 63;
     const int tx = tile % a.gx, ty = tile / a.gx;
     const uint2 range = a.ranges[tile];
     if (range.y <= range.x) return;
     const size_t HW = (size_t)a.H * a.W;
-    const float bg0 = a.bg[0], bg1 = a.bg[1], bg2 = a.bg[2];
 
     const int qx0i = tx * TILE + (wave & 1) * SUB, qy0i = ty * TILE + (wave >> 1) * SUB;
     const int pxi = qx0i + (lane & 7), pyi = qy0i + (lane >> 3);
     const bool inside = pxi < a.W && pyi < a.H;
     const size_t pix = (size_t)pyi * a.W + pxi;
     const float pxf = (float)pxi, pyf = (float)pyi;
-    const float T_final = inside ? final_T[pix] : 0.f;
     const uint32_t last = inside ? n_contrib[pix] : 0u;
+    const uint32_t maxc = (uint32_t)__builtin_amdgcn_readfirstlane((int)wave_max_u32(last));
+    if (maxc == 0) return;
+    const uint32_t m = DIR == 0 ? 0u : bs_split_point(maxc, sp);
+    if (FRONT && m == 0) return;
     const float g0 = inside ? dL_dcolor[pix] : 0.f;
     const float g1 = inside ? dL_dcolor[HW + pix] : 0.f;
     const float g2 = inside ? dL_dcolor[2 * HW + pix] : 0.f;
     const float gd = inside ? dL_ddepth[pix] : 0.f;
-    const float bgT = -T_final * (bg0 * g0 + bg1 * g1 + bg2 * g2);
-    float T = T_final, Bk = 0.f;
-    const uint32_t maxc = (uint32_t)__builtin_amdgcn_readfirstlane((int)wave_max_u32(last));
-    if (maxc == 0) return;
-    const uint32_t end = range.x + maxc;
+    float T, Bk, bgT = 0.f;
+    if (FRONT) {
+        const float C0 = inside ? out_color[pix] : 0.f, C1 = inside ? out_color[HW + pix] : 0.f;
+        const float C2 = inside ? out_color[2 * HW + pix] : 0.f, Dz = inside ? out_depth[pix] : 0.f;
+        T = 1.f;
+        Bk = -(C0 * g0 + C1 * g1 + C2 * g2 + Dz * gd);
+    } else {
+        const float T_final = inside ? final_T[pix] : 0.f;
+        bgT = -T_final * (a.bg[0] * g0 + a.bg[1] * g1 + a.bg[2] * g2);
+        T = T_final, Bk = 0.f;
+    }
+    const uint32_t end = range.x + (FRONT ? m : maxc);
+    const int b_lo = (int)(m / WAVE);
 #ifdef BS_TRACE
     unsigned long long tr0;
     uint32_t tr_n = 0;
@@ -793,19 +809,19 @@
             const bool in_i = (fxi + i) < a.W && fyi < a.H;
             const size_t px_i = (size_t)fyi * a.W + fxi + i;
             if (!POSE_ONLY) {
-                s_pix[ws][0][q][i] = in_i ? dL_dcolor[px_i] : 0.f;
-                s_pix[ws][1][q][i] = in_i ? dL_dcolor[HW + px_i] : 0.f;
-                s_pix[ws][2][q][i] = in_i ? dL_dcolor[2 * HW + px_i] : 0.f;
+                s_pix_ws[(0 * 16 + q) * 4 + i] = in_i ? dL_dcolor[px_i] : 0.f;
+                s_pix_ws[(1 * 16 + q) * 4 + i] = in_i ? dL_dcolor[HW + px_i] : 0.f;
+                s_pix_ws[(2 * 16 + q) * 4 + i] = in_i ? dL_dcolor[2 * HW + px_i] : 0.f;
             }
-            s_pix[ws][POSE_ONLY ? 0 : 3][q][i] = in_i ? dL_ddepth[px_i] : 0.f;
+            s_pix_ws[((POSE_ONLY ? 0 : 3) * 16 + q) * 4 + i] = in_i ? dL_ddepth[px_i] : 0.f;
         }
     }
     const int slot = POSE_ONLY ? bt_slot6(q) : bt_slot10(q);
     const uint32_t slot_bytes = slot < 0 ? 0u : (uint32_t)slot * 4u;
     const unsigned long long m_out = __builtin_amdgcn_ballot_w64(slot >= 0);
     const unsigned long long m_q0 = __builtin_amdgcn_ballot_w64((q & 3) == 0), m_q1 = __builtin_amdgcn_ballot_w64((q & 3) == 1);
-    const BtLane bl{&s_w[ws].h[0][0], &s_pix[ws][0][0][0], &s_w[ws].meta[0][0], lane, 0.f, 0.f, slot_bytes, m_out, m_q0, m_q1, grad_acc, qx0i, qy0i};
-    const uint32_t wbase = (uint32_t)__builtin_amdgcn_readfirstlane((int)(uint32_t)(uintptr_t)&s_w[ws]);
+    const BtLane bl{&s_w_ws->h[0][0], s_pix_ws, &s_w_ws->meta[0][0], lane, 0.f, 0.f, slot_bytes, m_out, m_q0, m_q1, grad_acc, qx0i, qy0i};
+    const uint32_t wbase = (uint32_t)__builtin_amdgcn_readfirstlane((int)(uint32_t)(uintptr_t)s_w_ws);
     const const_float_p recs = MGS_CONST(reinterpret_cast<const float*>(a.rec));
     uint32_t koff = 0;
     float zero = 0.f;
@@ -816,23 +832,24 @@
     auto prefetch = [&](int b) {
         gid_n = 0;
         box_n = make_float4(0.f, 0.f, -1.f, -1.f);
-        const uint32_t i = range.x + (uint32_t)b * WAVE + (uint32_t)(63 - lane);
-        if (b >= 0 && i < end) {
+        const uint32_t i = range.x + (uint32_t)b * WAVE + (uint32_t)(FRONT ? lane : 63 - lane);
+        if (b >= (FRONT ? 0 : b_lo) && i < end) {
             gid_n = a.point_list[i];
             box_n = a.rec[(size_t)gid_n * 4];
             ell_n = a.rec[(size_t)gid_n * 4 + 3];
         }
     };
-    prefetch((int)((maxc - 1) / WAVE));
-    for (int b = (int)((maxc - 1) / WAVE); b >= 0; --b) {
+    const int b_first = FRONT ? 0 : (int)((maxc - 1) / WAVE), b_step = FRONT ? 1 : -1;
+    prefetch(b_first);
+    for (int b = b_first; FRONT ? b < b_lo : b >= b_lo; b += b_step) {
         const float4 c = box_n, el = ell_n;
         v3f meta = {c.x, c.y, __uint_as_float(gid_n << 6)};
-        prefetch(b - 1);
+        prefetch(b + b_step);
         const unsigned long long alive = __builtin_amdgcn_ballot_w64(last >= (uint32_t)b * WAVE + 1u);
         int qxs = qx0i, qys = qy0i;
         asm volatile("" : "+s"(qxs), "+s"(qys));
         unsigned long long mask = __builtin_amdgcn_ballot_w64(quadrant_hit(c, el, (float)qxs, (float)qys, alive));
-        const int thr = 63 + (int)((uint32_t)b * WAVE + 1u) - (int)last;
+        const int thr = FRONT ? (int)last - (int)((uint32_t)b * WAVE + 1u) : 63 + (int)((uint32_t)b * WAVE + 1u) - (int)last;
 #define BS_POP(J, R0, R1)                                                                                                    \
         asm volatile("s_ff1_i32_b64 %0, %1\n\ts_bitset0_b64 %1, %0" : "=&s"(J), "+s"(mask));                                 \
         {                                                                                                                    \
@@ -843,6 +860,51 @@
         auto evaluate = [&](const v2f r0, const v8f r1, const int j) {
                 float dx, dy, t1, t2, G, al, inv, qq;
                 uint32_t adv, sa, tmp;
+                if (FRONT)
+                asm volatile(
+                    "v_sub_f32_e32 %[dx], %[px], %[pxf]\n\t"
+                    "v_sub_f32_e32 %[dy], %[py], %[pyf]\n\t"
+                    "v_mul_f32_e32 %[t1], %[cb], %[dy]\n\t"
+                    "v_mul_f32_e32 %[t2], %[cc], %[dy]\n\t"
+                    "v_fmac_f32_e32 %[t1], %[ca], %[dx]\n\t"
+                    "v_mul_f32_e32 %[t2], %[dy], %[t2]\n\t"
+                    "v_fmac_f32_e32 %[t2], %[dx], %[t1]\n\t"
+                    "v_exp_f32_e32 %[G], %[t2]\n\t"
+                    "s_add_u32 %[tmp], %[wbase], %[koff]\n\t"
+                    "v_lshl_add_u32 %[sa], %[lane], 2, %[tmp]\n\t"
+                    "ds_write2st64_b32 %[sa], %[zero], %[zero] offset1:5\n\t"
+                    "v_cmpx_le_i32_e32 vcc, %[j], %[thr]\n\t"
+                    "v_cmpx_nlt_f32_e32 vcc, 0, %[t2]\n\t"
+                    "v_mul_f32_e32 %[al], %[op], %[G]\n\t"
+                    "v_min_f32_e32 %[al], 0x3f7d70a4, %[al]\n\t"
+                    "v_cmpx_ngt_f32_e32 vcc, %[amin], %[al]\n\t"
+                    "v_sub_f32_e32 %[t1], 1.0, %[al]\n\t"
+                    "v_rcp_f32_e32 %[inv], %[t1]\n\t"
+                    "v_mul_f32_e32 %[qq], %[cr], %[g0]\n\t"
+                    "v_fmac_f32_e32 %[qq], %[cg], %[g1]\n\t"
+                    "v_fmac_f32_e32 %[qq], %[cb2], %[g2]\n\t"
+                    "v_fmac_f32_e32 %[qq], %[cz], %[gd]\n\t"
+                    "v_mul_f32_e32 %[dy], %[al], %[T]\n\t"
+                    "v_mul_f32_e32 %[dx], %[T], %[qq]\n\t"
+                    "v_fmac_f32_e32 %[Bk], %[dy], %[qq]\n\t"
+                    "v_fmac_f32_e32 %[dx], %[Bk], %[inv]\n\t"
+                    "v_mul_f32_e32 %[dx], %[G], %[dx]\n\t"
+                    "v_mul_f32_e32 %[T], %[T], %[t1]\n\t"
+                    "ds_write2st64_b32 %[sa], %[dx], %[dy] offset1:5\n\t"
+                    "s_cmp_lg_u64 exec, 0\n\t"
+                    "s_cselect_b32 %[adv], 272, 0\n\t"
+                    "s_lshl_b64 exec, 1, %[j]\n\t"
+                    "v_mov_b32_e32 %[sa], %[tmp]\n\t"
+                    "ds_write_b96 %[sa], %[meta] offset:2368\n\t"
+                    "s_mov_b64 exec, -1\n\t"
+                    : [dx] "=&v"(dx), [dy] "=&v"(dy), [t1] "=&v"(t1), [t2] "=&v"(t2), [G] "=&v"(G), [al] "=&v"(al), [inv] "=&v"(inv),
+                      [qq] "=&v"(qq), [sa] "=&v"(sa), [T] "+v"(T), [Bk] "+v"(Bk), [adv] "=&s"(adv), [tmp] "=&s"(tmp)
+                    : [px] "s"(r0[0]), [py] "s"(r0[1]), [ca] "s"(r1[0]), [cb] "s"(r1[1]), [cc] "s"(r1[2]), [op] "s"(r1[3]),
+                      [cr] "s"(r1[4]), [cg] "s"(r1[5]), [cb2] "s"(r1[6]), [cz] "s"(r1[7]), [pxf] "v"(pxf), [pyf] "v"(pyf), [thr] "v"(thr),
+                      [j] "s"(j), [g0] "v"(g0), [g1] "v"(g1), [g2] "v"(g2), [gd] "v"(gd), [lane] "v"(lane), [zero] "v"(zero),
+                      [koff] "s"(koff), [wbase] "s"(wbase), [meta] "v"(meta), [amin] "s"(1.0f / 255.0f)
+                    : "vcc", "scc", "memory");
+                else
                 asm volatile(
                     "v_sub_f32_e32 %[dx], %[px], %[pxf]\n\t"
                     "v_sub_f32_e32 %[dy], %[py], %[pyf]\n\t"
@@ -923,11 +985,42 @@
         BS_STAMP(tr1);
         const unsigned hw = __builtin_amdgcn_s_getreg((31 << 11) | 4), xcc = __builtin_amdgcn_s_getreg((31 << 11) | 20);
         if (lane == 0) {
-            unsigned long long* o = a.trace + ((size_t)tile * 4 + wave) * 4;
+            unsigned long long* o = a.trace + ((size_t)job * 4 + wave) * 4;
             o[0] = tr0; o[1] = tr1; o[2] = (unsigned long long)hw | ((unsigned long long)xcc << 32); o[3] = tr_n;
         }
     }
 #endif
+}
+
+template <bool POSE_ONLY, bool SPLIT>
+__global__ void __launch_bounds__(256) blend_backward_s_kernel(BlendArgs a, int ntiles,
+                                                               const float* __restrict__ final_T,
+                                                               const uint32_t* __restrict__ n_contrib,
+                                                               const float* __restrict__ dL_dcolor,
+                                                               const float* __restrict__ dL_ddepth,
+                                                               const float* __restrict__ out_color,
+                                                               const float* __restrict__ out_depth,
+                                                               float* __restrict__ grad_acc, BsSplit sp, int adjacent) {
+    __shared__ __attribute__((aligned(16))) BsWaveLds s_w[MGS_WG_WAVES];
+    __shared__ __attribute__((aligned(16))) float s_pix[MGS_WG_WAVES][POSE_ONLY ? 1 : 4][16][4];
+    const int wave = __builtin_amdgcn_readfirstlane((int)(threadIdx.x >> 6));
+    if (!SPLIT) {
+        const int tile = (int)blockIdx.x;
+        if (tile >= ntiles) return;
+        bs_walk<POSE_ONLY, 0>(a, tile, tile, wave, &s_w[wave], &s_pix[wave][0][0][0], final_T, n_contrib, dL_dcolor, dL_ddepth,
+                              out_color, out_depth, grad_acc, sp);
+    } else {
+        const int blk = (int)blockIdx.x;
+        if (blk >= 2 * ntiles) return;
+        const bool front = adjacent ? (blk & 1) != 0 : blk >= ntiles;
+        const int tile = adjacent ? blk >> 1 : (front ? blk - ntiles : blk);
+        if (front)
+            bs_walk<POSE_ONLY, 2>(a, tile, tile + ntiles, wave, &s_w[wave], &s_pix[wave][0][0][0], final_T, n_contrib, dL_dcolor,
+                                  dL_ddepth, out_color, out_depth, grad_acc, sp);
+        else
+            bs_walk<POSE_ONLY, 1>(a, tile, tile, wave, &s_w[wave], &s_pix[wave][0][0][0], final_T, n_contrib, dL_dcolor, dL_ddepth,
+                                  out_color, out_depth, grad_acc, sp);
+    }
 }
 
 __global__ void __launch_bounds__(256) blend_backward_stats_kernel(BlendArgs a, int ntiles,
@@ -1088,10 +1181,17 @@
 }
 
 int g_opt_blend_lds_pad_fwd = 0, g_opt_blend_lds_pad_bwd = 0;
+int g_opt_blend_bwd_split = -1;
+int g_opt_blend_bwd_split_min = BS_SPLIT_MIN, g_opt_blend_bwd_split_frac = BS_SPLIT_FRAC;
 int g_opt_blend_bwd_transposed = 2;
+int g_dbg_last_bwd_split = -1;
+static int bs_split_default(int ntiles, uint64_t num_rendered) {
+    return num_rendered >= (uint64_t)ntiles * 128u ? 1 : 0;
+}
+bool g_opt_blend_bwd_transposed_set = false;
 int launch_blend_backward(const mgs_camera& cam, const GeometryState& g, const BinningState& b,
-                          const ImageState& img, const float* dL_dcolor, const float* dL_ddepth, float* grad_acc,
-                          bool pose_only, hipStream_t s) {
+                          const ImageState& img, const float* dL_dcolor, const float* dL_ddepth, const float* out_color,
+                          const float* out_depth, float* grad_acc, bool pose_only, uint64_t num_rendered, hipStream_t s) {
     BlendArgs a = make_args(cam, g, b, img);
 #ifdef BS_TRACE
     a.trace = g_trace_bwd;
@@ -1099,13 +1199,20 @@
     const int ntiles = a.gx * tiles_y(a.H);
     if (ntiles == 0) return 0;
     if (g_opt_blend_bwd_transposed == 2) {
-        const dim3 grid(ntiles), block(256);
-        if (pose_only)
-            hipLaunchKernelGGL((blend_backward_s_kernel<true>), grid, block, (size_t)g_opt_blend_lds_pad_bwd, s, a, ntiles, img.final_T,
-                               img.n_contrib, dL_dcolor, dL_ddepth, grad_acc);
-        else
-            hipLaunchKernelGGL((blend_backward_s_kernel<false>), grid, block, (size_t)g_opt_blend_lds_pad_bwd, s, a, ntiles, img.final_T,
-                               img.n_contrib, dL_dcolor, dL_ddepth, grad_acc);
+        const int opt = g_opt_blend_bwd_split >= 0 ? g_opt_blend_bwd_split : g_opt_blend_bwd_transposed_set ? 0 : bs_split_default(ntiles, num_rendered);
+        bool split = opt != 0 && out_color && out_depth;
+#ifdef BS_TRACE
+        if (a.trace && g_trace_bwd_records < 8ull * (unsigned long long)ntiles) split = false;
+#endif
+        g_dbg_last_bwd_split = split ? 1 : 0;
+        const BsSplit sp{max(g_opt_blend_bwd_split_min, 2), min(max(g_opt_blend_bwd_split_frac, 1), 255)};
+        const dim3 grid(split ? 2 * ntiles : ntiles), block(256);
+        const size_t pad = (size_t)g_opt_blend_lds_pad_bwd;
+#define BS_LAUNCH(P_, S_) hipLaunchKernelGGL((blend_backward_s_kernel<P_, S_>), grid, block, pad, s, a, ntiles, img.final_T, img.n_contrib, \
+                                             dL_dcolor, dL_ddepth, out_color, out_depth, grad_acc, sp, (int)(opt == 2))
+        if (pose_only) { if (split) BS_LAUNCH(true, true); else BS_LAUNCH(true, false); }
+        else { if (split) BS_LAUNCH(false, true); else BS_LAUNCH(false, false); }
+#undef BS_LAUNCH
     } else if (g_opt_blend_bwd_transposed != 0) {
         if (pose_only)
             hipLaunchKernelGGL((blend_backward_t_kernel<true>), dim3(ntiles), dim3(256), 0, s, a, ntiles, img.final_T,
@@ -1141,9 +1248,10 @@
 }
 
 #ifdef BS_TRACE
-extern "C" int mgs_trace_set_blend_buffers(void* fwd, void* bwd) {
+extern "C" int mgs_trace_set_blend_buffers(void* fwd, void* bwd, unsigned long long bwd_records) {
     mgs::g_trace_fwd = (unsigned long long*)fwd;
     mgs::g_trace_bwd = (unsigned long long*)bwd;
+    mgs::g_trace_bwd_records = bwd ? bwd_records : 0;
     return 0;
 }
 #endif
diff --git a/monogs_amd/csrc/common.h b/monogs_amd/csrc/common.h
--- a/monogs_amd/csrc/common.h
+++ b/monogs_amd/csrc/common.h
@@ -217,14 +217,16 @@
 int launch_tile_depth_sort(const mgs_camera& cam, const TileSortArgs& ts, const ImageState& img, const uint32_t* sort_err,
                            hipStream_t s);
 int set_radix_spin_limit(uint32_t limit);
-extern int g_opt_radix_ballot_rank, g_opt_radix_scanned, g_opt_radix_xcd_band, g_opt_radix_tile_items, g_opt_knn_grid_min, g_opt_scan_small, g_opt_dup_slot_major, g_opt_blend_bwd_transposed, g_opt_blend_lds_pad_fwd, g_opt_blend_lds_pad_bwd, g_opt_depth_small;
+extern bool g_opt_blend_bwd_transposed_set;
+extern int g_dbg_last_bwd_split;
+extern int g_opt_radix_ballot_rank, g_opt_radix_scanned, g_opt_radix_xcd_band, g_opt_radix_tile_items, g_opt_knn_grid_min, g_opt_scan_small, g_opt_dup_slot_major, g_opt_blend_bwd_transposed, g_opt_blend_bwd_split, g_opt_blend_bwd_split_min, g_opt_blend_bwd_split_frac, g_opt_blend_lds_pad_fwd, g_opt_blend_lds_pad_bwd, g_opt_depth_small;
 int launch_blend_forward(const mgs_camera& cam, const GeometryState& g, const BinningState& b,
                          const ImageState& img, float* out_color, float* out_depth, float* out_opacity,
                          int32_t* n_touched, const uint32_t* sort_err, uint32_t* status, const TileSortArgs* tile_sort,
                          hipStream_t s);
 int launch_blend_backward(const mgs_camera& cam, const GeometryState& g, const BinningState& b,
-                          const ImageState& img, const float* dL_dcolor, const float* dL_ddepth,
-                          float* grad_acc, bool pose_only, hipStream_t s);
+                          const ImageState& img, const float* dL_dcolor, const float* dL_ddepth, const float* out_color,
+                          const float* out_depth, float* grad_acc, bool pose_only, uint64_t num_rendered, hipStream_t s);
 int launch_blend_backward_stats(const mgs_camera& cam, const GeometryState& g, const BinningState& b,
                                 const ImageState& img, unsigned long long* stats, hipStream_t s);
 int launch_valu_ceiling(float* out, int iters, hipStream_t s);
diff --git a/monogs_amd/rasterizer.py b/monogs_amd/rasterizer.py
--- a/monogs_amd/rasterizer.py
+++ b/monogs_amd/rasterizer.py
@@ -2,6 +2,7 @@
 
 import contextlib
 import ctypes as C
+import weakref
 from typing import NamedTuple, Optional
 
 import torch
@@ -229,6 +230,7 @@
             ctx.scratch_used = False
             out5 = torch.empty(5, H, W, dtype=torch.float32, device=dev)
             color, depth, opacity = out5[0:3], out5[3:4], out5[4:5]
+            ctx.out_ref = weakref.ref(out5) if want_bwd else None
             status = torch.empty(1, dtype=torch.int32, device=dev) if P > 0 else None
             key = (P, W, H)
             capturing = torch.cuda.is_current_stream_capturing()
@@ -296,6 +298,7 @@
         ctx.save_for_backward(means3D, sh_ if sh_ is not None else dummy, col_ if col_ is not None else dummy,
                               opac_, sc_ if sc_ is not None else dummy, rot_ if rot_ is not None else dummy,
                               cov_ if cov_ is not None else dummy, radii, arena, binning)
+        ctx.out_version = out5._version
         ctx.mark_non_differentiable(radii, n_touched)
         ctx.set_materialize_grads(False)
         return color, radii, depth, opacity, n_touched
@@ -340,12 +343,17 @@
                 d_tau = torch.empty(6, **f32) if want_tau else None
             timing = _lib.MgsTiming() if _timing_sink is not None else None
             tref = C.byref(timing) if timing is not None else None
+            out5 = ctx.out_ref() if ctx.out_ref is not None else None
+            if out5 is not None and out5._version != ctx.out_version:
+                out5 = None
             _lib.check(lib.mgs_backward(
                 C.byref(cam), P, ctx.num_rendered,
                 _ptr(means3D), _ptr(sh_) if has_sh else None, _ptr(col_) if has_col else None, _ptr(opac_),
                 _ptr(sc_) if has_sr else None, _ptr(rot_) if has_sr else None, _ptr(cov_) if has_cov else None,
                 radii.data_ptr(), geom_p, binning.data_ptr(), img_p,
                 g_color.data_ptr(), g_depth.data_ptr(),
+                out5.data_ptr() if out5 is not None else None,
+                out5.data_ptr() + 12 * H * W if out5 is not None else None,
                 _ptr(d_means2D), _ptr(d_col), _ptr(d_opac), _ptr(d_means3D), _ptr(d_cov), _ptr(d_sh),
                 _ptr(d_scales), _ptr(d_rot), _ptr(d_tau), scratch.data_ptr(), 1 if prepared else 0, tref, _stream()),
                 "mgs_backward")
```

Result: faster. 2949 Mpix/s (median of 6 runs) (+2.5%).
